# yweweler/single-speaker-tts

Hardware: AMD Instinct MI355X
Metric: mel-frames/sec (end-to-end text->waveform incl. 60-iter Griffin-Lim, 64-utt LJ-Speech-shaped batch per GPU) (higher is better)
Workload: dtype f32

## Files before the change

### include/sstts_hip.h

```cpp
#ifndef SSTTS_HIP_H
#define SSTTS_HIP_H

#include <stddef.h>
#include <stdint.h>

#ifdef __cplusplus
extern "C" {
#endif

typedef struct tts_handle_s* tts_handle_t;

enum tts_status {
    TTS_OK = 0,
    TTS_ERR_INVALID = -1,
    TTS_ERR_NOT_LOADED = -2,
    TTS_ERR_HIP = -3,
    TTS_ERR_DB_RANGE = -4,
    TTS_ERR_UNSUPPORTED = -5
};

typedef struct tts_config {
    int32_t struct_size;
    int32_t vocabulary_size;
    int32_t embedding_size;
    int32_t enc_prenet_units[2];
    int32_t enc_n_banks;
    int32_t enc_n_filters;
    int32_t enc_proj_filters[2];
    int32_t post_n_banks;
    int32_t post_n_filters;
    int32_t post_proj_filters[2];
    int32_t n_highway_layers;
    int32_t n_highway_units;
    int32_t n_gru_units;
    int32_t dec_prenet_units[2];
    int32_t n_attention_units;
    int32_t n_decoder_gru_units;
    int32_t n_decoder_gru_layers;
    int32_t n_mels;
    int32_t reduction;
    int32_t n_fft;
    int32_t force_cudnn;
    int32_t attention_mechanism;
    int32_t luong_local_window_d;
    int32_t luong_force_gaussian;
    int32_t luong_local_mode;
    int32_t apply_post_processing;
} tts_config_t;

enum tts_attention { TTS_ATTENTION_LUONG = 0, TTS_ATTENTION_LOCAL_LUONG = 1 };
enum tts_local_mode { TTS_LOCAL_MONOTONIC = 0, TTS_LOCAL_PREDICTIVE = 1 };

const char* tts_version(void);
int tts_default_config(tts_config_t* cfg);
int tts_create(const tts_config_t* cfg, int device_id, tts_handle_t* out);
int tts_destroy(tts_handle_t h);
const char* tts_last_error(tts_handle_t h);
int tts_set_stream(tts_handle_t h, void* hip_stream);
int tts_set_option(tts_handle_t h, const char* key, int value);
int tts_synchronize(tts_handle_t h);


int tts_manifest_size(tts_handle_t h);
int tts_manifest_entry(tts_handle_t h, int index, const char** name, int64_t shape[4], int* ndim);
int tts_set_weight(tts_handle_t h, const char* name, const float* host_data, const int64_t* shape, int ndim);
int tts_load_weights_blob(tts_handle_t h, const float* host_blob, size_t n_floats);
int tts_finalize_weights(tts_handle_t h);

int tts_malloc(void** dptr, size_t bytes);
int tts_free(void* dptr);
int tts_device_malloc(tts_handle_t h, void** dptr, size_t bytes);
int tts_device_free(tts_handle_t h, void* dptr);
int tts_memcpy_h2d(tts_handle_t h, void* dst, const void* src, size_t bytes);
int tts_memcpy_d2h(tts_handle_t h, void* dst, const void* src, size_t bytes);
int tts_memset(tts_handle_t h, void* dst, int value, size_t bytes);

int tts_encoder_forward(tts_handle_t h, const int32_t* ids, int B, int Ts, float* memory);
int tts_decoder_forward(tts_handle_t h, const float* memory, int B, int Ts, int n_steps,
                        float* mel, float* alignments);
int tts_postnet_forward(tts_handle_t h, const float* mel, int B, int T, float* linear);

int tts_evaluate(tts_handle_t h, const int32_t* ids, int B, int Ts, int n_steps,
                 const float* mel_target, const float* linear_target, float* losses,
                 double* l1_sums, float* mel, float* alignments, float* linear);

int tts_decoder_forward_teacher(tts_handle_t h, const float* memory, int B, int Ts, int n_steps,
                                const float* mel_target, float* mel, float* alignments);
int tts_teacher_forced(tts_handle_t h, const int32_t* ids, int B, int Ts, int n_steps,
                       const float* mel_target, const float* linear_target, float* losses,
                       double* l1_sums, float* mel, float* alignments, float* linear);
int tts_teacher_kernel_choice(tts_handle_t h, int B, int T_sent);

int tts_denorm_power(tts_handle_t h, const float* linear, int B, int T, int F,
                     float ref_db, float max_db, float power, float* mag);

int tts_griffin_lim(tts_handle_t h, const float* mag, const float* init_phase, uint64_t seed,
                    int B, int T, int n_iter, int win_length, int hop_length, int n_fft,
                    float* wav, float* mse);
int tts_griffin_lim_ragged(tts_handle_t h, const float* mag, const float* init_phase, uint64_t seed, int B, int T_max,
                           const int32_t* n_frames, int n_iter, int win_length, int hop_length, int n_fft,
                           float* wav, float* mse);
int tts_peak_normalize(tts_handle_t h, float* wav, int B, int n);

int tts_stft(tts_handle_t h, const float* wav, int B, int n, int n_fft, int win_length,
             int hop_length, float* out);
int tts_stft_magnitude(tts_handle_t h, const float* wav, int B, int n, int n_fft, int win_length,
                       int hop_length, float power, float* lin);
int tts_mel_spectrogram(tts_handle_t h, const float* lin, int B, int n_frames, int n_fft,
                        int sampling_rate, int n_mels, float fmin, float fmax, float* mel);
int tts_db_convert(tts_handle_t h, const float* in, size_t n, int mode, float ref_db, float max_db,
                   float* out);

int tts_trim_bounds(tts_handle_t h, const float* wav, const int64_t* offsets, int B, int frame_length, int hop_length,
                    float top_db, int64_t* bounds);

typedef struct tts_feature_params {
    int32_t struct_size;
    int32_t n_fft;
    int32_t win_length;
    int32_t hop_length;
    int32_t sampling_rate;
    int32_t n_mels;
    float fmin, fmax;
    float mel_ref_db, mel_max_db;
    float linear_ref_db, linear_max_db;
    int32_t normalize;
    int32_t reduction;
    int32_t trim;
    float trim_top_db;
    int32_t trim_frame_length;
    int32_t trim_hop_length;
} tts_feature_params_t;
int tts_default_feature_params(tts_feature_params_t* p);
int tts_plan_features(tts_handle_t h, const float* wav, const int64_t* offsets, int B, const tts_feature_params_t* p,
                      int64_t* plan);
int tts_extract_features(tts_handle_t h, const float* wav, const int64_t* offsets, int B, const tts_feature_params_t* p,
                         const int64_t* plan, float* mel_out, float* lin_out);

typedef struct tts_synth_params {
    int32_t n_steps;
    float ref_db, max_db;
    float power;
    int32_t n_iter;
    int32_t win_length, hop_length;
    uint64_t seed;
    int32_t peak_normalize;
    int32_t host_outputs;
} tts_synth_params_t;
#define TTS_HOST_LINEAR 1
#define TTS_HOST_ALIGNMENTS 2
int tts_synthesize(tts_handle_t h, const int32_t* ids, int B, int Ts, const tts_synth_params_t* p,
                   const float* init_phase , float* wav, float* mel,
                   float* alignments, float* linear);

int tts_synthesize_host(tts_handle_t h, const int32_t* ids_host, int B, int Ts, const tts_synth_params_t* p,
                        int* ticket);
int tts_wait_host(tts_handle_t h, int ticket, const float** wav_host, size_t* n_floats);
int tts_wait_host_outputs(tts_handle_t h, int ticket, const float** linear_host, size_t* n_linear, const float** align_host,
                          size_t* n_align);

int tts_profile_reset(tts_handle_t h);
int tts_decoder_kernel_choice(tts_handle_t h, int B, int T_sent, int pipelined);
int tts_debug_workspace(tts_handle_t h, const char* name, void** dptr, size_t* bytes);
int tts_debug_gl_plan(int T, int B, int win_length, int hop_length, int n_workers, int* items, int max_items, int* ring_frames);
int tts_debug_gl_plan_ragged(const int32_t* n_frames, int B, int win_length, int hop_length, int n_workers,
                             int* items, int max_items, int* ring_frames);
int tts_debug_gemm(tts_handle_t h, const float* A, const float* Wt, float* C, int M, int N, int Cin, int ktaps, int T,
                   int pool);
int tts_debug_hold(tts_handle_t h, int n_wgs, int lds_kb, double ms);
int tts_profile_get(tts_handle_t h, const char* stage, float* ms_total, int64_t* launches);
int tts_device_info(tts_handle_t h, char uuid_hex[33], int* n_compute_units);

#ifdef __cplusplus
}
#endif
#endif
```

### single-speaker-tts_amd/_hip.py

```python
import ctypes
import os
from ctypes import (POINTER, byref, c_char_p, c_float, c_int, c_int32, c_int64, c_size_t, c_uint64,
                    c_void_p)

import numpy as np

_HERE = os.path.dirname(os.path.abspath(__file__))
LIB_PATH = os.environ.get('SSTTS_HIP_LIB') or os.path.join(_HERE, 'libsstts_hip.so')

TTS_OK = 0
TTS_ERR_INVALID = -1
TTS_ERR_NOT_LOADED = -2
TTS_ERR_HIP = -3
TTS_ERR_DB_RANGE = -4
TTS_ERR_UNSUPPORTED = -5


class TtsError(RuntimeError):
    def __init__(self, code, msg):
        super().__init__('sstts_hip error {}: {}'.format(code, msg))
        self.code = code


class TtsConfig(ctypes.Structure):
    _fields_ = [
        ('struct_size', c_int32),
        ('vocabulary_size', c_int32), ('embedding_size', c_int32), ('enc_prenet_units', c_int32 * 2),
        ('enc_n_banks', c_int32), ('enc_n_filters', c_int32), ('enc_proj_filters', c_int32 * 2),
        ('post_n_banks', c_int32), ('post_n_filters', c_int32), ('post_proj_filters', c_int32 * 2),
        ('n_highway_layers', c_int32), ('n_highway_units', c_int32), ('n_gru_units', c_int32),
        ('dec_prenet_units', c_int32 * 2), ('n_attention_units', c_int32),
        ('n_decoder_gru_units', c_int32), ('n_decoder_gru_layers', c_int32), ('n_mels', c_int32),
        ('reduction', c_int32), ('n_fft', c_int32), ('force_cudnn', c_int32),
        ('attention_mechanism', c_int32), ('luong_local_window_d', c_int32), ('luong_force_gaussian', c_int32),
        ('luong_local_mode', c_int32), ('apply_post_processing', c_int32),
    ]


class TtsSynthParams(ctypes.Structure):
    _fields_ = [
        ('n_steps', c_int32), ('ref_db', c_float), ('max_db', c_float), ('power', c_float),
        ('n_iter', c_int32), ('win_length', c_int32), ('hop_length', c_int32), ('seed', c_uint64),
        ('peak_normalize', c_int32), ('host_outputs', c_int32),
    ]


class TtsFeatureParams(ctypes.Structure):
    _fields_ = [
        ('struct_size', c_int32), ('n_fft', c_int32), ('win_length', c_int32), ('hop_length', c_int32),
        ('sampling_rate', c_int32), ('n_mels', c_int32), ('fmin', c_float), ('fmax', c_float),
        ('mel_ref_db', c_float), ('mel_max_db', c_float), ('linear_ref_db', c_float), ('linear_max_db', c_float),
        ('normalize', c_int32), ('reduction', c_int32), ('trim', c_int32), ('trim_top_db', c_float),
        ('trim_frame_length', c_int32), ('trim_hop_length', c_int32),
    ]


_PROTOTYPES = {
    'tts_version': (c_char_p, []),
    'tts_default_config': (c_int, [POINTER(TtsConfig)]),
    'tts_create': (c_int, [POINTER(TtsConfig), c_int, POINTER(c_void_p)]),
    'tts_destroy': (c_int, [c_void_p]),
    'tts_last_error': (c_char_p, [c_void_p]),
    'tts_set_stream': (c_int, [c_void_p, c_void_p]),
    'tts_set_option': (c_int, [c_void_p, c_char_p, c_int]),
    'tts_synchronize': (c_int, [c_void_p]),
    'tts_manifest_size': (c_int, [c_void_p]),
    'tts_manifest_entry': (c_int, [c_void_p, c_int, POINTER(c_char_p), POINTER(c_int64), POINTER(c_int)]),
    'tts_set_weight': (c_int, [c_void_p, c_char_p, c_void_p, POINTER(c_int64), c_int]),
    'tts_load_weights_blob': (c_int, [c_void_p, c_void_p, c_size_t]),
    'tts_finalize_weights': (c_int, [c_void_p]),
    'tts_malloc': (c_int, [POINTER(c_void_p), c_size_t]),
    'tts_free': (c_int, [c_void_p]),
    'tts_device_malloc': (c_int, [c_void_p, POINTER(c_void_p), c_size_t]),
    'tts_device_free': (c_int, [c_void_p, c_void_p]),
    'tts_memcpy_h2d': (c_int, [c_void_p, c_void_p, c_void_p, c_size_t]),
    'tts_memcpy_d2h': (c_int, [c_void_p, c_void_p, c_void_p, c_size_t]),
    'tts_memset': (c_int, [c_void_p, c_void_p, c_int, c_size_t]),
    'tts_encoder_forward': (c_int, [c_void_p, c_void_p, c_int, c_int, c_void_p]),
    'tts_decoder_forward': (c_int, [c_void_p, c_void_p, c_int, c_int, c_int, c_void_p, c_void_p]),
    'tts_postnet_forward': (c_int, [c_void_p, c_void_p, c_int, c_int, c_void_p]),
    'tts_evaluate': (c_int, [c_void_p, c_void_p, c_int, c_int, c_int, c_void_p, c_void_p, c_void_p, c_void_p, c_void_p,
                             c_void_p, c_void_p]),
    'tts_decoder_forward_teacher': (c_int, [c_void_p, c_void_p, c_int, c_int, c_int, c_void_p, c_void_p, c_void_p]),
    'tts_teacher_forced': (c_int, [c_void_p, c_void_p, c_int, c_int, c_int, c_void_p, c_void_p, c_void_p, c_void_p,
                                   c_void_p, c_void_p, c_void_p]),
    'tts_teacher_kernel_choice': (c_int, [c_void_p, c_int, c_int]),
    'tts_denorm_power': (c_int, [c_void_p, c_void_p, c_int, c_int, c_int, c_float, c_float, c_float, c_void_p]),
    'tts_griffin_lim': (c_int, [c_void_p, c_void_p, c_void_p, c_uint64, c_int, c_int, c_int, c_int, c_int,
                                c_int, c_void_p, c_void_p]),
    'tts_griffin_lim_ragged': (c_int, [c_void_p, c_void_p, c_void_p, c_uint64, c_int, c_int, POINTER(c_int32), c_int, c_int,
                                       c_int, c_int, c_void_p, c_void_p]),
    'tts_peak_normalize': (c_int, [c_void_p, c_void_p, c_int, c_int]),
    'tts_stft': (c_int, [c_void_p, c_void_p, c_int, c_int, c_int, c_int, c_int, c_void_p]),
    'tts_db_convert': (c_int, [c_void_p, c_void_p, c_size_t, c_int, c_float, c_float, c_void_p]),
    'tts_stft_magnitude': (c_int, [c_void_p, c_void_p, c_int, c_int, c_int, c_int, c_int, c_float, c_void_p]),
    'tts_mel_spectrogram': (c_int, [c_void_p, c_void_p, c_int, c_int, c_int, c_int, c_int, c_float, c_float,
                                    c_void_p]),
    'tts_trim_bounds': (c_int, [c_void_p, c_void_p, c_void_p, c_int, c_int, c_int, c_float, c_void_p]),
    'tts_default_feature_params': (c_int, [POINTER(TtsFeatureParams)]),
    'tts_plan_features': (c_int, [c_void_p, c_void_p, c_void_p, c_int, POINTER(TtsFeatureParams), c_void_p]),
    'tts_extract_features': (c_int, [c_void_p, c_void_p, c_void_p, c_int, POINTER(TtsFeatureParams), c_void_p, c_void_p,
                                     c_void_p]),
    'tts_synthesize': (c_int, [c_void_p, c_void_p, c_int, c_int, POINTER(TtsSynthParams), c_void_p, c_void_p,
                               c_void_p, c_void_p, c_void_p]),
    'tts_synthesize_host': (c_int, [c_void_p, c_void_p, c_int, c_int, POINTER(TtsSynthParams), POINTER(c_int)]),
    'tts_wait_host': (c_int, [c_void_p, c_int, POINTER(c_void_p), POINTER(c_size_t)]),
    'tts_wait_host_outputs': (c_int, [c_void_p, c_int, POINTER(c_void_p), POINTER(c_size_t), POINTER(c_void_p), POINTER(c_size_t)]),
    'tts_profile_reset': (c_int, [c_void_p]),
    'tts_profile_get': (c_int, [c_void_p, c_char_p, POINTER(c_float), POINTER(c_int64)]),
    'tts_decoder_kernel_choice': (c_int, [c_void_p, c_int, c_int, c_int]),
    'tts_debug_workspace': (c_int, [c_void_p, c_char_p, POINTER(c_void_p), POINTER(c_size_t)]),
    'tts_debug_hold': (c_int, [c_void_p, c_int, c_int, ctypes.c_double]),
    'tts_debug_gemm': (c_int, [c_void_p, c_void_p, c_void_p, c_void_p, c_int, c_int, c_int, c_int, c_int, c_int]),
    'tts_debug_gl_plan': (c_int, [c_int, c_int, c_int, c_int, c_int, POINTER(c_int), c_int, POINTER(c_int)]),
    'tts_debug_gl_plan_ragged': (c_int, [POINTER(c_int32), c_int, c_int, c_int, c_int, POINTER(c_int), c_int, POINTER(c_int)]),
    'tts_device_info': (c_int, [c_void_p, c_char_p, POINTER(c_int)]),
}

_lib = None


def exported_symbols():
    return sorted(_PROTOTYPES)


def load_library(path=None):
    global _lib
    if _lib is not None and path is None:
        return _lib
    path = path or LIB_PATH
    if not os.path.exists(path):
        raise OSError('{} not found: build it with `python single-speaker-tts_amd/build.py` '
                      '(there is no CPU fallback)'.format(path))
    lib = ctypes.CDLL(path)
    for name, (res, args) in _PROTOTYPES.items():
        fn = getattr(lib, name)
        fn.restype = res
        fn.argtypes = args
    _lib = lib
    return lib


class DeviceArray(object):

    def __init__(self, engine, shape, dtype=np.float32):
        self.engine = engine
        self.shape = tuple(int(s) for s in shape)
        self.dtype = np.dtype(dtype)
        self.nbytes = int(np.prod(self.shape, dtype=np.int64)) * self.dtype.itemsize
        p = c_void_p()
        rc = engine.lib.tts_device_malloc(engine.handle, byref(p), self.nbytes)
        if rc != TTS_OK:
            raise TtsError(rc, 'tts_device_malloc({}) failed'.format(self.nbytes))
        self.ptr = p.value

    def data_ptr(self):
        return self.ptr

    def copy_from(self, host):
        host = np.ascontiguousarray(host, dtype=self.dtype)
        assert host.nbytes == self.nbytes, (host.shape, self.shape)
        self.engine._check(self.engine.lib.tts_memcpy_h2d(self.engine.handle, self.ptr, host.ctypes.data,
                                                          self.nbytes))
        return self

    def to_host(self):
        out = np.empty(self.shape, dtype=self.dtype)
        self.engine._check(self.engine.lib.tts_memcpy_d2h(self.engine.handle, out.ctypes.data, self.ptr,
                                                          self.nbytes))
        return out

    def free(self):
        if self.ptr:
            if getattr(self.engine, 'handle', None):
                self.engine.lib.tts_device_free(self.engine.handle, self.ptr)
            else:
                self.engine.lib.tts_free(self.ptr)
            self.ptr = None

    def __del__(self):
        try:
            self.free()
        except Exception:
            pass


def _is_device(x):
    return hasattr(x, 'data_ptr') and not isinstance(x, np.ndarray)


def ragged_frame_counts(n_frames, B, T_max, hop_length, n_fft):
    nf = np.ascontiguousarray(np.asarray(n_frames).reshape(-1), dtype=np.int32)
    if nf.shape[0] != B:
        raise ValueError('n_frames: {} lengths for a batch of {}'.format(nf.shape[0], B))
    for b, n in enumerate(nf.tolist()):
        if not 1 <= n <= T_max:
            raise ValueError('n_frames[{}] = {} is not in 1 .. T_max = {}'.format(b, n, T_max))
        if hop_length * (n - 1) <= n_fft // 2:
            raise ValueError('n_frames[{}] = {}: the signal is shorter than n_fft / 2 (reflect padding undefined)'.format(b, n))
    return nf


def momentum_thousandths(momentum):
    m = float(momentum)
    if not 0.0 <= m < 1.0:
        raise ValueError('momentum must be in [0, 1), got {!r}'.format(momentum))
    return min(999, int(round(m * 1000.0)))


class _MomentumScope(object):

    def __init__(self, engine, momentum):
        self.engine = engine
        self.value = None if momentum is None else momentum_thousandths(momentum)

    def __enter__(self):
        self.saved = self.engine._gl_momentum
        if self.value is not None and self.value != self.saved:
            self.engine.set_option('gl_momentum', self.value)

    def __exit__(self, *exc):
        if self.engine._gl_momentum != self.saved:
            self.engine.set_option('gl_momentum', self.saved)
        return False


class Engine(object):

    def __init__(self, hparams=None, device_id=0, stream=None):
        self.lib = load_library()
        cfg = TtsConfig()
        self.lib.tts_default_config(byref(cfg))
        if hparams is not None:
            enc, dec, post = hparams.encoder, hparams.decoder, hparams.post
            cfg.vocabulary_size = hparams.vocabulary_size
            cfg.embedding_size = enc.embedding_size
            cfg.enc_prenet_units[0], cfg.enc_prenet_units[1] = [l[0] for l in enc.pre_net_layers]
            cfg.enc_n_banks, cfg.enc_n_filters = enc.n_banks, enc.n_filters
            cfg.enc_proj_filters[0], cfg.enc_proj_filters[1] = [p[0] for p in enc.projections]
            cfg.post_n_banks, cfg.post_n_filters = post.n_banks, post.n_filters
            cfg.post_proj_filters[0], cfg.post_proj_filters[1] = [p[0] for p in post.projections]
            cfg.n_highway_layers, cfg.n_highway_units = enc.n_highway_layers, enc.n_highway_units
            cfg.n_gru_units = enc.n_gru_units
            cfg.dec_prenet_units[0], cfg.dec_prenet_units[1] = [l[0] for l in dec.pre_net_layers]
            cfg.n_attention_units = dec.n_attention_units
            cfg.n_decoder_gru_units = dec.n_decoder_gru_units
            cfg.n_decoder_gru_layers = dec.n_gru_layers
            cfg.n_mels, cfg.reduction, cfg.n_fft = hparams.n_mels, hparams.reduction, hparams.n_fft
            cfg.force_cudnn = 1 if hparams.force_cudnn else 0
            att = hparams.attention
            if att.mechanism not in ('LuongAttention', 'LocalLuongAttention'):
                raise NotImplementedError('attention mechanism {!r}'.format(att.mechanism))
            if att.mechanism == 'LocalLuongAttention' and (att.luong_local_mode not in ('monotonic', 'predictive') or
                                                           att.luong_local_score != 'dot'):
                raise NotImplementedError('LocalLuongAttention: the general / concat scores raise '
                                          'NotImplementedError in the reference too')
            cfg.luong_local_mode = 1 if att.luong_local_mode == 'predictive' else 0
            cfg.attention_mechanism = 1 if att.mechanism == 'LocalLuongAttention' else 0
            cfg.luong_local_window_d = att.luong_local_window_D
            cfg.luong_force_gaussian = 1 if att.luong_force_gaussian else 0
            cfg.apply_post_processing = 1 if hparams.apply_post_processing else 0
        self.cfg = cfg
        h = c_void_p()
        rc = self.lib.tts_create(byref(cfg), device_id, byref(h))
        if rc != TTS_OK:
            raise TtsError(rc, (self.lib.tts_last_error(None) or b'').decode())
        self.handle = h
# ... 412 lines not shown
```

### single-speaker-tts_amd/csrc/api_handle.hip

```cpp
#include "api_internal.h"

namespace tts_api {
thread_local std::string g_create_error;
const char* const kStageNames[ST_COUNT] = {"encoder", "decoder", "postnet", "denorm", "gl_iter", "gl_final", "debug_gemm", "eval_loss", "features"};
}

namespace tts_api {


int fail(tts_handle_t h, int code, const std::string& msg) {
    if (h) h->err = msg;
    else g_create_error = msg;
    return code;
}


const char* kAtt = "decoder2/decoder/output_projection_wrapper/multi_rnn_cell/cell_0/attention_wrapper";

const char* kMrc = "decoder2/decoder/output_projection_wrapper/multi_rnn_cell";


std::string bn_name(int i) {
    return i == 0 ? std::string("batch_normalization") : "batch_normalization_" + std::to_string(i);
}
// ... 179 lines not shown
        const auto& bh = W(h, hs + "/H/bias");
        const auto& bt = W(h, hs + "/T/bias");
        const size_t ow = p.alloc((size_t)2 * U * U);
        const size_t ob = p.alloc((size_t)2 * U);
        for (int u = 0; u < U; ++u) {
            const int s = u / 32, w = u % 32;
            const int rh = 64 * s + w, rt = 64 * s + 32 + w;
            for (int k = 0; k < U; ++k) {
                p.host[ow + (size_t)rh * U + k] = kh[(size_t)k * U + u];
                p.host[ow + (size_t)rt * U + k] = kt[(size_t)k * U + u];
            }
            p.host[ob + rh] = bh[u];
            p.host[ob + rt] = bt[u];
        }
        o.hw_wt.push_back(ow);
        o.hw_b.push_back(ob);
    }
    const int H = c.n_gru_units;
    o.gru_in_wt = p.alloc((size_t)6 * H * U);
    o.gru_in_b = p.alloc((size_t)6 * H);
    o.gru_rec = p.alloc(bigru_wrec_floats(H, cudnn));
    const size_t rec_stride = bigru_wrec_floats(H, cudnn) / 2;
    const char* dirs[2] = {"fw", "bw"};
    for (int d = 0; d < 2; ++d) {
        const std::string gs = scope + "/gru/" + dirs[d] + "/gru_cell_" + dirs[d];
        const auto& gk = W(h, gs + "/gates/kernel");
        const auto& gb = W(h, gs + "/gates/bias");
        const float* ck_in;
        int ck_in_ld;
        const float* ck_h;
        const float* cb;
        if (cudnn) {
            ck_in = W(h, gs + "/candidate/input_projection/kernel").data();
            ck_h = W(h, gs + "/candidate/hidden_projection/kernel").data();
            cb = W(h, gs + "/candidate/input_projection/bias").data();
        } else {
            ck_in = W(h, gs + "/candidate/kernel").data();
            ck_h = ck_in + (size_t)U * H;
            cb = W(h, gs + "/candidate/bias").data();
        }
        ck_in_ld = H;
        float* wt = p.host.data() + o.gru_in_wt + (size_t)d * 3 * H * U;
        float* bb = p.host.data() + o.gru_in_b + (size_t)d * 3 * H;
        for (int n = 0; n < 2 * H; ++n) {
            for (int k = 0; k < U; ++k) wt[(size_t)n * U + k] = gk[(size_t)k * 2 * H + n];
            bb[n] = gb[n];
        }
        for (int n = 0; n < H; ++n) {
            for (int k = 0; k < U; ++k) wt[(size_t)(2 * H + n) * U + k] = ck_in[(size_t)k * ck_in_ld + n];
            bb[2 * H + n] = cb[n];
        }
        float* rec = p.host.data() + o.gru_rec + (size_t)d * rec_stride;
        for (int k = 0; k < H; ++k)
            for (int n = 0; n < 2 * H; ++n) rec[(size_t)k * 2 * H + n] = gk[(size_t)(U + k) * 2 * H + n];
        float* rc = rec + (size_t)H * 2 * H;
        for (int k = 0; k < H; ++k)
            for (int n = 0; n < H; ++n) rc[(size_t)k * H + n] = ck_h[(size_t)k * H + n];
        if (cudnn) {
            const auto& hb = W(h, gs + "/candidate/hidden_projection/bias");
            for (int n = 0; n < H; ++n) rc[(size_t)H * H + n] = hb[n];
        }
    }
    return o;
}


void bind_cbhg(CbhgWeights& w, const CbhgOffsets& o, const float* base, int n_in, int n_banks, int n_filters,
               const int proj[2]) {
    w.n_banks = n_banks;
    w.n_filters = n_filters;
    w.c_in = n_in;
    w.proj_filters[0] = proj[0];
    w.proj_filters[1] = proj[1];
    for (int k = 0; k < n_banks; ++k) {
        w.bank_wt.push_back(base + o.bank_wt[k]);
        w.bank_b.push_back(base + o.bank_b[k]);
        w.bank_scale.push_back(base + o.bank_scale[k]);
        w.bank_shift.push_back(base + o.bank_shift[k]);
    }
    for (int i = 0; i < 2; ++i) {
        w.proj_wt[i] = base + o.proj_wt[i];
        w.proj_b[i] = base + o.proj_b[i];
        w.proj_scale[i] = base + o.proj_scale[i];
        w.proj_shift[i] = base + o.proj_shift[i];
    }
    w.lifter_wt = base + o.lifter_wt;
    w.lifter_b = base + o.lifter_b;
    for (size_t l = 0; l < o.hw_wt.size(); ++l) {
        w.hw_wt.push_back(base + o.hw_wt[l]);
        w.hw_b.push_back(base + o.hw_b[l]);
    }
    w.gru_in_wt = base + o.gru_in_wt;
    w.gru_in_b = base + o.gru_in_b;
    w.gru_rec = base + o.gru_rec;
}


struct GruOffsets {
    size_t gates_wt, gates_b, cand_wt, cand_b;
};


GruOffsets pack_dec_gru(tts_handle_t h, Packer& p, const std::string& scope, int n_in, int U, bool cudnn) {
    GruOffsets o{};
    const auto& gk = W(h, scope + "/gates/kernel");
    const auto& gb = W(h, scope + "/gates/bias");
    const int K = n_in + U;
    if (!cudnn) {
        o.gates_wt = pack_transposed(p, gk.data(), K, 2 * U);
        o.gates_b = pack_copy(p, gb.data(), 2 * U);
        o.cand_wt = pack_transposed(p, W(h, scope + "/candidate/kernel").data(), K, U);
        o.cand_b = pack_copy(p, W(h, scope + "/candidate/bias").data(), U);
        return o;
    }
    const auto& ik = W(h, scope + "/candidate/input_projection/kernel");
    const auto& ib = W(h, scope + "/candidate/input_projection/bias");
    const auto& hk = W(h, scope + "/candidate/hidden_projection/kernel");
    const auto& hb = W(h, scope + "/candidate/hidden_projection/bias");
    o.gates_wt = p.alloc((size_t)4 * U * K);
    o.gates_b = p.alloc((size_t)4 * U);
    float* wt = p.host.data() + o.gates_wt;
    float* bb = p.host.data() + o.gates_b;
    for (int n = 0; n < 2 * U; ++n) {
        for (int k = 0; k < K; ++k) wt[(size_t)n * K + k] = gk[(size_t)k * 2 * U + n];
        bb[n] = gb[n];
    }
    for (int n = 0; n < U; ++n) {
        for (int k = 0; k < U; ++k) wt[(size_t)(2 * U + n) * K + n_in + k] = hk[(size_t)k * U + n];
        bb[2 * U + n] = hb[n];
        for (int k = 0; k < n_in; ++k) wt[(size_t)(3 * U + n) * K + k] = ik[(size_t)k * U + n];
        bb[3 * U + n] = ib[n];
    }
    o.cand_wt = o.gates_wt;
    o.cand_b = o.gates_b;
    return o;
}


int pd_timed_out(tts_handle_t h) {
    return fail(h, TTS_ERR_HIP,
                "persistent decoder: a workgroup waited for its cluster longer than the bound (not all "
                "workgroups were co-resident); the outputs of that call are invalid -- the handle has "
                "switched to the launch-per-layer path (tts_set_option(h, \"persistent_decoder\", 1) switches back)");
}

int check_status(tts_handle_t h) {
    if (h->pd_used) {
        h->pd_used = false;
        int status = 0;
        HIPCHK(h, hipMemcpy(&status, h->pd_sync + 64 * h->pd_clusters + 1, sizeof(int), hipMemcpyDeviceToHost));
        if (status) HIPCHK(h, hipMemset(h->pd_sync + 64 * h->pd_clusters + 1, 0, sizeof(int)));
        if (status) h->persistent_decoder = 0;
        if (status) return pd_timed_out(h);
    }
    return TTS_OK;
}


int sync_all(tts_handle_t h) {
    HIPCHK(h, hipStreamSynchronize(h->stream));
    if (h->pl.front && h->pl.front != h->stream) HIPCHK(h, hipStreamSynchronize(h->pl.front));
    if (h->pl.aux) HIPCHK(h, hipStreamSynchronize(h->pl.aux));
    if (h->pl.encs) HIPCHK(h, hipStreamSynchronize(h->pl.encs));
    if (h->hio.out) HIPCHK(h, hipStreamSynchronize(h->hio.out));
    return check_status(h);
}


int graph_quiesce(tts_handle_t h) {
    HIPCHK(h, h->graph_done.sync());
    h->graph_done.disarm();
    return TTS_OK;
}

int graph_drop(tts_handle_t h) {
    if (h->dec_graph) {
        int rc = graph_quiesce(h);
        if (rc) return rc;
        hipGraphExecDestroy(h->dec_graph);
        h->dec_graph = nullptr;
    }
    if (h->dec_graph_src) {
        hipGraphDestroy(h->dec_graph_src);
        h->dec_graph_src = nullptr;
    }
    return TTS_OK;
}


int ws_get(tts_handle_t h, const char* name, size_t bytes, void** out) {
    DevBuf& b = h->ws[name];
    if (b.bytes < bytes) {
        if (b.p) {
            {
                int rc = sync_all(h);
                if (rc) return rc;
            }
            HIPCHK(h, hipFree(b.p));
            b.p = nullptr;
            b.bytes = 0;
            {
                int rc = graph_drop(h);
                if (rc) return rc;
            }
        }
        HIPCHK(h, hipMalloc(&b.p, bytes));
        b.bytes = bytes;
    }
    *out = b.p;
    return TTS_OK;
}


void prof_collect(tts_handle_t h) {
    sync_all(h);
    if (!h->spans.empty() && h->debug_hooks && h->timeline) {
        for (auto& s : h->spans) {
            float t0 = 0.f, t1 = 0.f;
            if (hipEventElapsedTime(&t0, h->spans[0].a, s.a) == hipSuccess &&
                hipEventElapsedTime(&t1, h->spans[0].a, s.b) == hipSuccess)
                fprintf(stderr, "timeline %-8s %9.3f -> %9.3f ms (%.3f)\n", kStageNames[s.stage], t0, t1, t1 - t0);
        }
    }
    for (auto& s : h->spans) {
        float ms = 0.f;
        if (hipEventElapsedTime(&ms, s.a, s.b) == hipSuccess) {
            h->prof_ms[s.stage] += ms;
            h->prof_launches[s.stage] += s.launches;
        }
        hipEventDestroy(s.a);
        hipEventDestroy(s.b);
    }
    h->spans.clear();
}


GemmGroup dense_group(const float* A, int lda, const float* Wt, const float* bias, float* C, int ldc, int M, int N,
                      int K, int act) {
    GemmGroup g;
    std::memset(&g, 0, sizeof(g));
    g.A = A; g.Wt = Wt; g.bias = bias; g.C = C;
    g.M = M; g.N = N; g.K = K;
    g.lda = lda; g.T = M; g.Cin = K; g.padl = 0; g.pool = 0;
    g.ldc = ldc; g.coff = 0; g.act = act; g.epi = EPI_STD;
    return g;
}


GemmGroup conv_group(const float* A, int Cin, int ktaps, int T, const float* Wt, const float* bias,
                     const float* scale, const float* shift, float* C, int ldc, int coff, int M, int N, int act,
                     int pool) {
    GemmGroup g;
    std::memset(&g, 0, sizeof(g));
    g.A = A; g.Wt = Wt; g.bias = bias; g.scale = scale; g.shift = shift; g.C = C;
    g.M = M; g.N = N; g.K = ktaps * Cin;
    g.lda = Cin; g.T = T; g.Cin = Cin; g.padl = (ktaps - 1) / 2; g.pool = pool;
    g.ldc = ldc; g.coff = coff; g.act = act; g.epi = EPI_STD;
    return g;
}


int run_single(tts_handle_t h, const GemmGroup& g) {
    GemmBatch b;
    std::memset(&b, 0, sizeof(b));
    b.g[0] = g;
    HIPCHK(h, launch_gemm(h->stream, b, 1));
    return TTS_OK;
}


bool graph_runtime_ok(int* have) {
    int v = 0;
    if (hipRuntimeGetVersion(&v) != hipSuccess) v = 0;
    if (have) *have = v;
    return v / 100000 >= HIP_VERSION / 100000;
}

}

extern "C" {


const char* tts_version(void) { return "sstts_hip 0.1.0 (gfx950)"; }


int tts_default_config(tts_config_t* c) {
    if (!c) return TTS_ERR_INVALID;
    std::memset(c, 0, sizeof(*c));
    c->struct_size = (int32_t)sizeof(tts_config_t);
    c->vocabulary_size = 39;
    c->embedding_size = 256;
    c->enc_prenet_units[0] = 256; c->enc_prenet_units[1] = 128;
    c->enc_n_banks = 16; c->enc_n_filters = 128;
    c->enc_proj_filters[0] = 128; c->enc_proj_filters[1] = 128;
    c->post_n_banks = 8; c->post_n_filters = 128;
    c->post_proj_filters[0] = 256; c->post_proj_filters[1] = 80;
    c->n_highway_layers = 4; c->n_highway_units = 128; c->n_gru_units = 128;
    c->dec_prenet_units[0] = 256; c->dec_prenet_units[1] = 128;
    c->n_attention_units = 256; c->n_decoder_gru_units = 256; c->n_decoder_gru_layers = 2;
    c->n_mels = 80; c->reduction = 5; c->n_fft = 2048; c->force_cudnn = 0;
    c->attention_mechanism = TTS_ATTENTION_LUONG;
    c->luong_local_window_d = 10;
    c->luong_force_gaussian = 1;
    c->luong_local_mode = TTS_LOCAL_MONOTONIC;
    c->apply_post_processing = 1;
    return TTS_OK;
// ... 20 lines not shown
        !mult(c.enc_n_filters, 32) || !mult(c.post_n_filters, 32) || !mult(c.enc_proj_filters[0], 4) ||
        !mult(c.post_proj_filters[0], 4))
        return fail(nullptr, TTS_ERR_UNSUPPORTED, "layer widths must be multiples of 16 (filters: 32)");
    if (c.enc_proj_filters[1] != c.enc_prenet_units[1] || c.post_proj_filters[1] != c.n_mels)
        return fail(nullptr, TTS_ERR_INVALID, "last projection must match the CBHG input width (residual)");
    if (c.attention_mechanism != TTS_ATTENTION_LUONG && c.attention_mechanism != TTS_ATTENTION_LOCAL_LUONG)
        return fail(nullptr, TTS_ERR_UNSUPPORTED, "attention_mechanism must be TTS_ATTENTION_LUONG or TTS_ATTENTION_LOCAL_LUONG");
    if (c.attention_mechanism == TTS_ATTENTION_LOCAL_LUONG && c.luong_local_window_d < 1)
        return fail(nullptr, TTS_ERR_INVALID, "luong_local_window_d must be >= 1");
    if (c.luong_local_mode != TTS_LOCAL_MONOTONIC && c.luong_local_mode != TTS_LOCAL_PREDICTIVE)
        return fail(nullptr, TTS_ERR_INVALID, "luong_local_mode must be TTS_LOCAL_MONOTONIC or TTS_LOCAL_PREDICTIVE");
    if (c.enc_n_banks < 1 || c.post_n_banks < 1 || c.reduction < 1 || c.vocabulary_size < 1 || c.n_highway_layers < 0)
        return fail(nullptr, TTS_ERR_INVALID, "bad counts");
    if (c.n_mels > TTS_MAX_N_MELS)
        return fail(nullptr, TTS_ERR_UNSUPPORTED,
                    "n_mels is " + std::to_string(c.n_mels) + ", at most " + std::to_string(TTS_MAX_N_MELS) +
                    " supported (the decoder's GO frame is read from a block of that many zeros)");
    {
        const int fields[] = {c.vocabulary_size, c.embedding_size, c.enc_prenet_units[0], c.enc_prenet_units[1], c.enc_n_banks,
                              c.enc_n_filters, c.enc_proj_filters[0], c.enc_proj_filters[1], c.post_n_banks, c.post_n_filters,
                              c.post_proj_filters[0], c.post_proj_filters[1], c.dec_prenet_units[0], c.dec_prenet_units[1],
                              c.reduction, c.n_highway_layers};
        for (int v : fields)
            if (v > TTS_MAX_FIELD)
                return fail(nullptr, TTS_ERR_UNSUPPORTED, "a count or layer width of " + std::to_string(v) + ": at most " +
                                                              std::to_string(TTS_MAX_FIELD) + " (2^20) supported");
        struct { const char* what; long long n; } mats[] = {
            {"the embedding table (vocabulary_size x embedding_size)", (long long)c.vocabulary_size * c.embedding_size},
            {"encoder pre-net layer 1", (long long)c.embedding_size * c.enc_prenet_units[0]},
            {"encoder pre-net layer 2", (long long)c.enc_prenet_units[0] * c.enc_prenet_units[1]},
            {"the widest encoder bank convolution (enc_n_banks x enc_prenet_units[1] x enc_n_filters)",
             (long long)c.enc_n_banks * c.enc_prenet_units[1] * c.enc_n_filters},
            {"encoder projection 1 (3 x enc_n_banks x enc_n_filters x enc_proj_filters[0])",
             3ll * c.enc_n_banks * c.enc_n_filters * c.enc_proj_filters[0]},
            {"encoder projection 2", 3ll * c.enc_proj_filters[0] * c.enc_proj_filters[1]},
            {"the widest post-net bank convolution (post_n_banks x n_mels x post_n_filters)",
             c.apply_post_processing ? (long long)c.post_n_banks * c.n_mels * c.post_n_filters : 0},
            {"post-net projection 1 (3 x post_n_banks x post_n_filters x post_proj_filters[0])",
             c.apply_post_processing ? 3ll * c.post_n_banks * c.post_n_filters * c.post_proj_filters[0] : 0},
            {"post-net projection 2", c.apply_post_processing ? 3ll * c.post_proj_filters[0] * c.post_proj_filters[1] : 0},
            {"the output projection (n_decoder_gru_units x n_mels x reduction)",
             (long long)c.n_decoder_gru_units * c.n_mels * c.reduction}};
        for (const auto& m : mats)
            if (m.n > TTS_MAX_WEIGHT_FLOATS)
                return fail(nullptr, TTS_ERR_UNSUPPORTED,
                            std::string(m.what) + " has " + std::to_string(m.n) + " weights, at most " +
                            std::to_string(TTS_MAX_WEIGHT_FLOATS) + " (2^30 - 5) supported: the GEMM loaders address an operand "
                            "with 32-bit byte offsets");
    }
    if (hipSetDevice(device_id) != hipSuccess) return fail(nullptr, TTS_ERR_HIP, "hipSetDevice failed");
    auto h = new tts_handle_s();
    h->cfg = c;
    h->device = device_id;
    if (hipStreamCreate(&h->stream) != hipSuccess) {
        delete h;
        return fail(nullptr, TTS_ERR_HIP, "hipStreamCreate failed");
    }
    h->own_stream = true;
    {
        int cus = 0;
        if (hipDeviceGetAttribute(&cus, hipDeviceAttributeMultiprocessorCount, device_id) != hipSuccess || cus < 1) cus = 256;
        h->n_cus_dev = cus;
    }
    build_manifest(h);
    *out = h;
    return TTS_OK;
}


int tts_destroy(tts_handle_t h) {
    DeviceScope dev_scope(h);
    if (!h) return TTS_OK;
    hipSetDevice(h->device);
    hipStreamSynchronize(h->stream);
    for (auto& s : h->spans) {
        hipEventDestroy(s.a);
        hipEventDestroy(s.b);
    }
    graph_drop(h);
    for (auto& kv : h->ws)
        if (kv.second.p) hipFree(kv.second.p);
    if (h->arena) hipFree(h->arena);
    if (h->gl.window) hipFree(h->gl.window);
    if (h->gl.wss) hipFree(h->gl.wss);
    if (h->gl.wlane) hipFree(h->gl.wlane);
    if (h->gl.tw1024) hipFree(h->gl.tw1024);
    if (h->gl.tw2048) hipFree(h->gl.tw2048);
    if (h->gl.tables) hipFree(h->gl.tables);
    if (h->an.window) hipFree(h->an.window);
    if (h->an.mel_wt) hipFree(h->an.mel_wt);
    feat_release(h);
    if (h->an.flag) hipFree(h->an.flag);
    for (auto& kv : h->glg.tw) hipFree(kv.second);
    if (h->glg.window) hipFree(h->glg.window);
    if (h->glg.rwss) hipFree(h->glg.rwss);
    h->pl.teardown();
    h->hio.teardown();
    if (h->own_stream) hipStreamDestroy(h->stream);
    delete h;
    return TTS_OK;
}


const char* tts_last_error(tts_handle_t h) { return h ? h->err.c_str() : g_create_error.c_str(); }


int tts_set_stream(tts_handle_t h, void* s) {
    DeviceScope dev_scope(h);
    if (!h) return TTS_ERR_INVALID;
    {
        int rc = sync_all(h);
        if (rc) return rc;
    }
    h->pl.reset();
    {
        int rc = graph_drop(h);
        if (rc) return rc;
    }
    if (h->own_stream) hipStreamDestroy(h->stream);
    if (s) {
        h->stream = reinterpret_cast<hipStream_t>(s);
        h->own_stream = false;
    } else {
        HIPCHK(h, hipStreamCreate(&h->stream));
        h->own_stream = true;
    }
    return TTS_OK;
}


int tts_set_option(tts_handle_t h, const char* key, int value) {
    DeviceScope dev_scope(h);
    if (!h || !key) return TTS_ERR_INVALID;
    if (!std::strcmp(key, "use_graph")) {
        int have = 0;
        if (value && !(value == 2 && h->debug_hooks) && !graph_runtime_ok(&have))
            return fail(h, TTS_ERR_UNSUPPORTED,
                        "use_graph: this process runs the library on HIP runtime " + std::to_string(have) + ", older than the " +
                        std::to_string(HIP_VERSION) + " it was built with (a libamdhip64 loaded before the library, e.g. the one "
                        "PyTorch bundles); hipGraph replays of the decoder are wrong there (csrc/api_internal.h, `use_graph`) -- the "
                        "launches are enqueued directly instead");
        h->use_graph = value;
    }
    else if (!std::strcmp(key, "profile")) h->profile = value;
    else if (!std::strcmp(key, "fused_tail")) h->fused_tail = value;
    else if (!std::strcmp(key, "persistent_decoder")) {
        if (value != h->persistent_decoder) {
            int rc = sync_all(h);
            if (rc) return rc;
        }
        h->persistent_decoder = value;
    }
    else if (!std::strcmp(key, "gl_pair")) h->gl_pair = value;
    else if (!std::strcmp(key, "gl_momentum")) {
        if (value < 0 || value > 999) return fail(h, TTS_ERR_INVALID, "gl_momentum: thousandths of the momentum, 0 .. 999");
        h->gl_momentum = value;
    }
    else if (!std::strcmp(key, "gl_wide_from")) h->gl_wide = value < -2 ? -2 : value;
    else if (!std::strcmp(key, "pd_ws")) {
        if (value != h->pd_ws) {
            int rc = sync_all(h);
            if (rc) return rc;
        }
        h->pd_ws = value;
    }
    else if (!std::strcmp(key, "enc_stream")) {
        int rc = sync_all(h);
        if (rc) return rc;
        h->enc_stream = value;
    }
    else if (!std::strcmp(key, "debug_hooks")) h->debug_hooks = value;
    else if (!std::strcmp(key, "pd_debug_delay") || !std::strcmp(key, "gl_runs") || !std::strcmp(key, "gl_run_len") ||
             !std::strcmp(key, "timeline") || !std::strcmp(key, "gl_workers") || !std::strcmp(key, "pd_rows")) {
        if (!h->debug_hooks && value != 0)
            return fail(h, TTS_ERR_INVALID, std::string(key) + ": a test hook; set the option \"debug_hooks\" to 1 on this handle first");
        if (!std::strcmp(key, "pd_debug_delay")) h->pd_debug_delay = value;
        else if (!std::strcmp(key, "gl_runs")) h->gl_runs = value;
        else if (!std::strcmp(key, "gl_run_len")) h->gl_run_len = value;
        else if (!std::strcmp(key, "gl_workers")) h->gl_workers = value;
        else if (!std::strcmp(key, "pd_rows")) h->pd_rows = value;
        else h->timeline = value;
    }
    else if (!std::strcmp(key, "reserve_cus")) {
        if (value != h->reserve_cus) {
            int rc = sync_all(h);
            if (rc) return rc;
        }
        h->reserve_cus = value;
    } else if (!std::strcmp(key, "hold_lds_kb")) {
        if (value < 1 || value > 160) return fail(h, TTS_ERR_INVALID, "hold_lds_kb must be 1..160");
        h->hold_lds_kb = value;
    } else if (!std::strcmp(key, "pipeline")) {
        int rc = sync_all(h);
        if (rc) return rc;
        h->pl.reset();
        h->pipeline = value;
    }
    else return fail(h, TTS_ERR_INVALID, std::string("unknown option ") + key);
    return TTS_OK;
}


int tts_synchronize(tts_handle_t h) {
    DeviceScope dev_scope(h);
    if (!h) return TTS_ERR_INVALID;
    return sync_all(h);
}


int tts_manifest_size(tts_handle_t h) { return h ? (int)h->manifest.size() : TTS_ERR_INVALID; }


int tts_manifest_entry(tts_handle_t h, int i, const char** name, int64_t shape[4], int* ndim) {
    if (!h || i < 0 || i >= (int)h->manifest.size()) return TTS_ERR_INVALID;
    const auto& e = h->manifest[i];
    if (name) *name = e.name.c_str();
    if (ndim) *ndim = (int)e.shape.size();
    if (shape)
        for (size_t d = 0; d < 4; ++d) shape[d] = d < e.shape.size() ? e.shape[d] : 1;
    return TTS_OK;
}


int tts_set_weight(tts_handle_t h, const char* name, const float* data, const int64_t* shape, int ndim) {
    if (!h || !name || !data || !shape) return TTS_ERR_INVALID;
    for (const auto& e : h->manifest) {
        if (e.name != name) continue;
        if ((int)e.shape.size() != ndim) return fail(h, TTS_ERR_INVALID, std::string("rank mismatch for ") + name);
        for (int d = 0; d < ndim; ++d)
            if (e.shape[d] != shape[d]) return fail(h, TTS_ERR_INVALID, std::string("shape mismatch for ") + name);
        h->host_w[e.name].assign(data, data + e.numel());
        h->finalized = false;
        return TTS_OK;
    }
    return fail(h, TTS_ERR_INVALID, std::string("unknown weight ") + name);
}


int tts_load_weights_blob(tts_handle_t h, const float* blob, size_t n) {
    if (!h || !blob) return TTS_ERR_INVALID;
    size_t total = 0;
    for (const auto& e : h->manifest) total += e.numel();
    if (total != n)
        return fail(h, TTS_ERR_INVALID,
                    "blob has " + std::to_string(n) + " floats, manifest needs " + std::to_string(total));
    size_t off = 0;
    for (const auto& e : h->manifest) {
        h->host_w[e.name].assign(blob + off, blob + off + e.numel());
        off += e.numel();
    }
    h->finalized = false;
    return TTS_OK;
}


int tts_finalize_weights(tts_handle_t h) {
    DeviceScope dev_scope(h);
    if (!h) return TTS_ERR_INVALID;
    for (const auto& e : h->manifest)
        if (!h->host_w.count(e.name)) return fail(h, TTS_ERR_NOT_LOADED, "missing weight " + e.name);
    HIPCHK(h, hipSetDevice(h->device));
    const tts_config_t& c = h->cfg;
    const bool cudnn = c.force_cudnn != 0;
    Packer p;
    const size_t o_emb = pack_copy(p, W(h, "encoder/embedding").data(), (size_t)c.vocabulary_size * c.embedding_size);
    size_t o_epw[2], o_epb[2];
    int n_in = c.embedding_size;
    for (int i = 0; i < 2; ++i) {
        const std::string s = "encoder/pre_net/" + std::to_string(i + 1) + "-FC-" + std::to_string(c.enc_prenet_units[i]);
        o_epw[i] = pack_transposed(p, W(h, s + "/kernel").data(), n_in, c.enc_prenet_units[i]);
        o_epb[i] = pack_copy(p, W(h, s + "/bias").data(), c.enc_prenet_units[i]);
        n_in = c.enc_prenet_units[i];
    }
    const CbhgOffsets o_enc =
        pack_cbhg(h, p, "encoder", n_in, c.enc_n_banks, c.enc_n_filters, c.enc_proj_filters, cudnn);
    const int mem = 2 * c.n_gru_units, att = c.n_attention_units, U = c.n_decoder_gru_units;
    const size_t o_mem = pack_transposed(p, W(h, "decoder2/memory_layer/kernel").data(), mem, att);
    size_t o_dpw[2], o_dpb[2];
    n_in = c.n_mels + att;
    for (int i = 0; i < 2; ++i) {
        const std::string s = std::string(kAtt) + "/pre_net/" + std::to_string(i + 1) + "-FC-" +
                              std::to_string(c.dec_prenet_units[i]);
        o_dpw[i] = pack_transposed(p, W(h, s + "/kernel").data(), n_in, c.dec_prenet_units[i]);
        o_dpb[i] = pack_copy(p, W(h, s + "/bias").data(), c.dec_prenet_units[i]);
        n_in = c.dec_prenet_units[i];
    }
    size_t o_dpfw, o_dpfb;
    {
        const int NM = c.n_mels, OUTW = c.n_mels * c.reduction, P1 = c.dec_prenet_units[0];
        const std::string s1 = std::string(kAtt) + "/pre_net/1-FC-" + std::to_string(P1);
        const auto& w1 = W(h, s1 + "/kernel");
        const auto& b1 = W(h, s1 + "/bias");
        const auto& wo = W(h, "decoder2/decoder/output_projection_wrapper/kernel");
        const auto& bo = W(h, "decoder2/decoder/output_projection_wrapper/bias");
        const int K = U + att;
        o_dpfw = p.alloc((size_t)P1 * K);
        o_dpfb = p.alloc((size_t)P1);
        for (int n = 0; n < P1; ++n) {
            for (int k = 0; k < U; ++k) {
                double acc = 0.0;
                for (int j = 0; j < NM; ++j)
                    acc += (double)wo[(size_t)k * OUTW + (OUTW - NM) + j] * (double)w1[(size_t)j * P1 + n];
                p.host[o_dpfw + (size_t)n * K + k] = (float)acc;
            }
            for (int k = 0; k < att; ++k) p.host[o_dpfw + (size_t)n * K + U + k] = w1[(size_t)(NM + k) * P1 + n];
            double bacc = (double)b1[n];
            for (int j = 0; j < NM; ++j) bacc += (double)bo[(OUTW - NM) + j] * (double)w1[(size_t)j * P1 + n];
            p.host[o_dpfb + n] = (float)bacc;
        }
    }
    const GruOffsets o_ag = pack_dec_gru(h, p, std::string(kAtt) + "/gru_cell", n_in, att, cudnn);
    const size_t o_al = pack_transposed(p, W(h, std::string(kAtt) + "/attention_layer/kernel").data(), att + mem, att);
    const bool predictive = c.attention_mechanism == TTS_ATTENTION_LOCAL_LUONG && c.luong_local_mode == TTS_LOCAL_PREDICTIVE;
    size_t o_wp = 0, o_vp = 0;
    if (predictive) {
        o_wp = pack_copy(p, W(h, std::string(kAtt) + "/local_luong_attention/local_w_p").data(), (size_t)att * att);
        o_vp = pack_copy(p, W(h, std::string(kAtt) + "/local_luong_attention/local_v_p").data(), (size_t)att);
    }
    GruOffsets o_dg[4];
    for (int i = 0; i < c.n_decoder_gru_layers; ++i)
        o_dg[i] = pack_dec_gru(h, p, std::string(kMrc) + "/cell_" + std::to_string(i + 1) + "/gru_cell",
                               i == 0 ? att : U, U, cudnn);
    const int OUT = c.n_mels * c.reduction;
    const size_t o_ow = pack_transposed(p, W(h, "decoder2/decoder/output_projection_wrapper/kernel").data(), U, OUT);
    const size_t o_ob = pack_copy(p, W(h, "decoder2/decoder/output_projection_wrapper/bias").data(), OUT);
    CbhgOffsets o_post{};
    if (c.apply_post_processing)
        o_post = pack_cbhg(h, p, "post_process", c.n_mels, c.post_n_banks, c.post_n_filters, c.post_proj_filters, cudnn);
    const int F = 1 + c.n_fft / 2;
    const size_t o_dw = pack_transposed(p, W(h, "dense/kernel").data(), c.apply_post_processing ? mem : c.n_mels, F);
    const size_t o_db = pack_copy(p, W(h, "dense/bias").data(), F);
    const size_t o_zero = p.alloc(TTS_MAX_N_MELS);
    size_t o_wsw = 0, o_wsb = 0;
// ... 177 lines not shown
```

### single-speaker-tts_amd/csrc/api_internal.h

```cpp
#pragma once
#include <cmath>
#include <cstdio>
#include <cstring>
#include <memory>
#include <mutex>
#include <optional>
#include <string>
#include <utility>
#include <vector>
#include "decoder.h"
#include "griffin_lim.h"
#include "tts_common.h"
#include <algorithm>
#include <map>

namespace tts_api {
using namespace tts;


constexpr int TTS_MAX_N_MELS = 1024;
constexpr int TTS_MAX_FIELD = 1 << 20;
constexpr long long TTS_MAX_WEIGHT_FLOATS = (1ll << 30) - 5;

extern thread_local std::string g_create_error;
// ... 30 lines not shown
    hipEvent_t a, b;
    int stage;
    int64_t launches;
};

struct Signal {
    hipEvent_t ev = nullptr;
    bool armed = false;
    Signal() = default;
    Signal(const Signal&) = delete;
    Signal& operator=(const Signal&) = delete;
    ~Signal() {
        if (ev) hipEventDestroy(ev);
    }
    hipError_t record(hipStream_t s) {
        hipError_t e = ev ? hipSuccess : hipEventCreateWithFlags(&ev, hipEventDisableTiming);
        if (e == hipSuccess) e = hipEventRecord(ev, s);
        if (e == hipSuccess) armed = true;
        return e;
    }
    hipError_t wait(hipStream_t s) const { return armed ? hipStreamWaitEvent(s, ev, 0) : hipSuccess; }
    hipError_t sync() const { return armed ? hipEventSynchronize(ev) : hipSuccess; }
    void disarm() { armed = false; }
};

template <class T>
struct StagedBuf {
    T* pinned = nullptr;
    T* dev = nullptr;
    size_t bytes = 0;
    StagedBuf() = default;
    StagedBuf(const StagedBuf&) = delete;
    StagedBuf& operator=(const StagedBuf&) = delete;
    ~StagedBuf() { release(); }
    hipError_t release() {
        const hipError_t e1 = pinned ? hipHostFree(pinned) : hipSuccess;
        const hipError_t e2 = dev ? hipFree(dev) : hipSuccess;
        pinned = dev = nullptr;
        bytes = 0;
        return e1 != hipSuccess ? e1 : e2;
    }
    hipError_t grow(size_t need) {
        if (need <= bytes) return hipSuccess;
        hipError_t e = release();
        if (e == hipSuccess) e = hipHostMalloc(reinterpret_cast<void**>(&pinned), need, hipHostMallocDefault);
        if (e == hipSuccess) e = hipMalloc(reinterpret_cast<void**>(&dev), need);
        if (e == hipSuccess) bytes = need;
        return e;
    }
};

struct StageArgs {
    int* hold_flag = nullptr;
    int cu_budget = 0;
    bool chip_idle = false;
    bool project_later = false;
    int parity = 0;
    float* keys = nullptr;
    struct {
        int32_t* dst = nullptr;
        const int32_t* src = nullptr;
        size_t bytes = 0;
        Signal* done = nullptr;
    } upload;
    Signal* enc_done = nullptr;
};

struct CallPipeline {
    hipStream_t aux = nullptr;
    int* hold_flags = nullptr;
    Signal aux_mark;
    unsigned call_count = 0;
    hipStream_t front = nullptr;
    hipStream_t encs = nullptr;
    Signal enc_ready[2];
    Signal dec_done[2];
    Signal gap[2];
    Signal front_done;
    Signal post_done[2];
    bool gl_wide_used[2] = {false, false};
    Signal gl_done[2];
    Signal serial_done;
    unsigned syn_calls = 0;
    int syn_shape[3] = {0, 0, 0};
    int last_enc_ahead = -1;

    void reset() {
        for (Signal* s : {&aux_mark, &front_done, &serial_done}) s->disarm();
        for (int i = 0; i < 2; ++i) {
            for (Signal* s : {&enc_ready[i], &dec_done[i], &gap[i], &post_done[i], &gl_done[i]}) s->disarm();
            gl_wide_used[i] = false;
        }
    }
    void teardown() {
        for (hipStream_t s : {front, aux})
            if (s) {
                hipStreamSynchronize(s);
                hipStreamDestroy(s);
            }
        if (hold_flags) hipFree(hold_flags);
        if (encs) hipStreamDestroy(encs);
    }
};

struct HostIo {
    hipStream_t out = nullptr;
    StagedBuf<int32_t> ids[3];
    StagedBuf<float> wav[3];
    Signal h2d[3];
    Signal enc[3];
    Signal ready[3];
    Signal d2h[3];
    size_t n_floats[3] = {0, 0, 0};
    StagedBuf<float> lin[3], ali[3];
    size_t n_lin[3] = {0, 0, 0}, n_ali[3] = {0, 0, 0};
    bool failed[3] = {false, false, false};
    int* status_pinned = nullptr;
    int tickets = 0;

    void reset() {
        for (int i = 0; i < 3; ++i)
            for (Signal* s : {&h2d[i], &enc[i], &ready[i], &d2h[i]}) s->disarm();
    }
    void teardown() {
        if (status_pinned) hipHostFree(status_pinned);
        if (out) hipStreamDestroy(out);
    }
};

}
using namespace tts_api;

struct tts_handle_s {
    tts_config_t cfg;
    int device = 0;
    hipStream_t stream = nullptr;
    bool own_stream = false;
    std::string err;
    int use_graph = 0;
    int fused_tail = 1;
    bool tail_configured = false;
    int profile = 0;
    int pipeline = 1;
    int reserve_cus = 32;
    int hold_lds_kb = 64;
    int enc_stream = 1;
    CallPipeline pl;
    int persistent_decoder = 1;
    int pd_ws = 1;
    bool ws_configured = false;
    int gl_pair = 3;
    int gl_momentum = 0;
    int gl_wide = -1;
    int n_cus_dev = 0;
    bool pd_configured = false;
    int debug_hooks = 0;
    int pd_debug_delay = 0;
    int gl_runs = 0;
    int gl_run_len = 0;
    int timeline = 0;
    int gl_workers = 0;
    unsigned* gl_ring = nullptr;
    unsigned gl_ring_seq = 0;
    unsigned* gl_ring_last = nullptr;
    hipStream_t gl_ring_stream = nullptr;
    bool pd_used = false;
    unsigned* pd_sync = nullptr;
    int pd_clusters = 0;
    int pd_rows = 0;
    int pd_rows_used = 0;

    HostIo hio;

    std::vector<ManifestEntry> manifest;
    std::map<std::string, std::vector<float>> host_w;
    bool finalized = false;

    float* arena = nullptr;
    size_t arena_floats = 0;

    const float* embedding = nullptr;
    const float* enc_pre_wt[2];
    const float* enc_pre_b[2];
    CbhgWeights enc, post;
    const float* mem_wt = nullptr;
    DecoderWeights dec;
    const float* dense_wt = nullptr;
    const float* dense_b = nullptr;
    const float* zeros = nullptr;

    std::map<std::string, DevBuf> ws;

    hipGraphExec_t dec_graph = nullptr;
    Signal graph_done;
    hipGraph_t dec_graph_src = nullptr;
    struct {
        const void* memory = nullptr;
        const void* keys = nullptr;
        void* align = nullptr;
        int B = 0, Ts = 0, n_steps = 0;
        DecoderScratch sc;
        DecoderWeights w;
    } dec_key;

    struct {
        int win = 0, hop = 0, T = 0;
        float* window = nullptr;
        float* wss = nullptr;
        float* wlane = nullptr;
        float2* tw1024 = nullptr;
        float2* tw2048 = nullptr;
        float2* tables = nullptr;
        bool configured = false;
        int n_cus = 0;
    } gl;

    struct {
        std::map<int, float2*> tw;
        int n_fft = 0, win = 0, hop = 0, T = 0;
        float* window = nullptr;
        float* rwss = nullptr;
        bool configured = false;
    } glg;

    struct {
        std::vector<int> tab_key, plan_key;
        int* lens = nullptr;
        float* rw = nullptr;
        int4* items = nullptr;
        int n_items = 0, slots = 1, workers = 1;
    } rag;

    struct {
        int win = 0;
        float* window = nullptr;
        int sr = 0, n_fft = 0, n_mels = 0;
        float fmin = 0, fmax = 0;
        float* mel_wt = nullptr;
        int* flag = nullptr;
    } an;

    struct {
        int n_fft = 0, win = 0;
        float* window = nullptr;
        int sr = 0, n_mels = 0;
        float fmin = 0, fmax = 0;
        float* mel_w = nullptr;
        int* mel_band = nullptr;
        void* staging = nullptr;
        size_t staging_bytes = 0;
        Signal staged;
    } feat;

    std::vector<ProfSpan> spans;
    double prof_ms[ST_COUNT] = {0};
    int64_t prof_launches[ST_COUNT] = {0};
};


namespace tts_api {

#define HIPCHK(h, expr)                                                                         \
    do {                                                                                        \
        hipError_t _e = (expr);                                                                 \
        if (_e != hipSuccess) {                                                                 \
            (h)->err = std::string(#expr) + ": " + hipGetErrorString(_e);                       \
            return TTS_ERR_HIP;                                                                 \
        }                                                                                       \
    } while (0)

struct DeviceScope {
    int prev = -1;
    bool changed = false;
    explicit DeviceScope(tts_handle_t h) {
        if (!h) return;
        if (hipGetDevice(&prev) == hipSuccess && prev != h->device) changed = hipSetDevice(h->device) == hipSuccess;
    }
    ~DeviceScope() {
        if (changed) hipSetDevice(prev);
    }
    DeviceScope(const DeviceScope&) = delete;
    DeviceScope& operator=(const DeviceScope&) = delete;
};

#define WS(h, name, type, count, var)                                             \
    type* var = nullptr;                                                          \
    {                                                                             \
        void* _p = nullptr;                                                       \
        int _rc = ws_get(h, name, (size_t)(count) * sizeof(type), &_p);           \
        if (_rc != TTS_OK) return _rc;                                            \
        var = reinterpret_cast<type*>(_p);                                        \
    }

struct ProfScope {
    tts_handle_t h;
    int idx = -1;
    ProfScope(tts_handle_t h_, int stage, int64_t launches) : h(h_) {
        if (!h->profile) return;
        ProfSpan s{};
        if (hipEventCreate(&s.a) != hipSuccess || hipEventCreate(&s.b) != hipSuccess) return;
        s.stage = stage;
        s.launches = launches;
        hipEventRecord(s.a, h->stream);
        h->spans.push_back(s);
        idx = (int)h->spans.size() - 1;
    }
    ~ProfScope() {
        if (idx >= 0) hipEventRecord(h->spans[idx].b, h->stream);
    }
};

int fail(tts_handle_t h, int code, const std::string& msg);
void build_manifest(tts_handle_t h);
int pd_timed_out(tts_handle_t h);
// ... 41 lines not shown
```

### single-speaker-tts_amd/csrc/api_stages.hip

```cpp
#include "api_internal.h"

namespace tts_api {


int run_cbhg(tts_handle_t h, const CbhgWeights& w, const char* tag, const float* x, int B, int T, float* out,
             int64_t* launches) {
    const tts_config_t& c = h->cfg;
    const int M = B * T;
    const int NB = w.n_banks, NF = w.n_filters;
    const int U = c.n_highway_units, H = c.n_gru_units;
    const std::string t(tag);
    WS(h, (t + ".bank").c_str(), float, (size_t)M * NB * NF, bank);
    WS(h, (t + ".p1").c_str(), float, (size_t)M * w.proj_filters[0], p1);
    WS(h, (t + ".p2").c_str(), float, (size_t)M * w.proj_filters[1], p2);
    WS(h, (t + ".hw0").c_str(), float, (size_t)M * U, hw0);
    WS(h, (t + ".hw1").c_str(), float, (size_t)M * U, hw1);
    WS(h, (t + ".xproj").c_str(), float, (size_t)M * 6 * H, xproj);

    for (int k0 = 0; k0 < NB; k0 += TTS_GEMM_MAX_GROUPS) {
        GemmBatch b;
        std::memset(&b, 0, sizeof(b));
        const int ng = std::min(TTS_GEMM_MAX_GROUPS, NB - k0);
        for (int i = 0; i < ng; ++i) {
            const int k = k0 + ng - 1 - i;
// ... 335 lines not shown
        rwss = h->rag.rw;
    }
    const float2* tw = nullptr;
    if ((rc = glg_twiddles(h, n_fft, &tw))) return rc;
    const int F = 1 + n_fft / 2, Fp = gl_fp(n_fft), L = hop * (T - 1);
    WS(h, "glg.phase", float2, (size_t)B * T * Fp, ph);
    WS(h, "glg.frames", float, (size_t)B * T * win, frames);
    WS(h, "glg.mse_partial", float, (size_t)B * T, msep);
    const float alpha = (float)(h->gl_momentum / 1000.0);
    float2* mom_c = nullptr;
    if (h->gl_momentum > 0 && n_iter > 1) {
        WS(h, "glg.mom", float2, (size_t)B * T * Fp, mc);
        mom_c = mc;
    }
    float* sig = wav;
    HIPCHK(h, launch_glg_phase_init(h->stream, init_ft, seed, ph, B, F, T, Fp, d_lens));
    {
        ProfScope ps(h, ST_GL_ITER, 3 * (int64_t)n_iter);
        for (int it = 0; it < n_iter; ++it) {
            HIPCHK(h, launch_glg_istft(h->stream, mag_int, ph, h->glg.window, rwss, tw, frames, sig, B, T, Fp, n_fft, win, hop, d_lens));
            const bool want_mse = mse && it == n_iter - 1;
            HIPCHK(h, launch_glg_stft(h->stream, sig, L, h->glg.window, tw, ph, B, T, Fp, n_fft, win, hop, 0, mag_int,
                                      want_mse ? msep : nullptr, mom_c, alpha, it == 0, d_lens));
        }
    }
    if (mse) {
        if (n_iter > 0 && d_lens) HIPCHK(h, launch_gl_mse_reduce_ragged(h->stream, msep, B, T, F, d_lens, 1, mse));
        else if (n_iter > 0) HIPCHK(h, launch_gl_mse_reduce(h->stream, msep, B, T, (float)((double)F * T), mse));
        else HIPCHK(h, hipMemsetAsync(mse, 0, B * sizeof(float), h->stream));
    }
    {
        ProfScope ps(h, ST_GL_FINAL, 2);
        HIPCHK(h, launch_glg_istft(h->stream, mag_int, ph, h->glg.window, rwss, tw, frames, wav, B, T, Fp, n_fft, win, hop, d_lens));
    }
    if (peak_normalize) HIPCHK(h, launch_peak_normalize(h->stream, wav, B, L));
    return TTS_OK;
}


int gl_prepare(tts_handle_t h, int T, int win, int hop, int n_fft) {
    if (!gl_is_streaming(n_fft, win, hop)) return fail(h, TTS_ERR_UNSUPPORTED, "griffin_lim: the streaming kernel is instantiated for 1102 / 275 and 800 / 200 at n_fft 2048 only");
    if (win < 2 || win > n_fft || hop < 1 || T < 1)
        return fail(h, TTS_ERR_INVALID, "griffin_lim: need 2 <= win_length <= n_fft, hop_length >= 1, T >= 1");
    const int ncol = (win + hop - 1) / hop;
    if (ncol > 8) return fail(h, TTS_ERR_UNSUPPORTED, "griffin_lim: win_length / hop_length > 8 not supported");
    if ((long long)hop * (T - 1) <= n_fft / 2)
        return fail(h, TTS_ERR_INVALID, "griffin_lim: signal shorter than n_fft/2 (reflect padding undefined)");
    auto& g = h->gl;
    {
        int rc = gl_tables(h);
        if (rc) return rc;
    }
    if (g.win == win && g.hop == hop && g.T == T) return TTS_OK;
    HIPCHK(h, hipStreamSynchronize(h->stream));
    if (g.window) hipFree(g.window);
    if (g.wss) hipFree(g.wss);
    if (g.wlane) hipFree(g.wlane);
    g.window = g.wss = g.wlane = nullptr;
    std::vector<double> wd;
    std::vector<float> wf, wss;
    hann_window(win, wd, wf);
    recip_window_sumsquare(wd, n_fft, hop, T, wss);
    HIPCHK(h, hipMalloc(&g.window, win * sizeof(float)));
    HIPCHK(h, hipMalloc(&g.wss, wss.size() * sizeof(float)));
    HIPCHK(h, hipMemcpy(g.window, wf.data(), win * sizeof(float), hipMemcpyHostToDevice));
    HIPCHK(h, hipMemcpy(g.wss, wss.data(), wss.size() * sizeof(float), hipMemcpyHostToDevice));
    {
        std::vector<float> wl(2 * 16 * 2 * 64);
        gl_build_wlane(wf.data(), wss.data(), win, hop, T, wl.data());
        HIPCHK(h, hipMalloc(&g.wlane, wl.size() * sizeof(float)));
        HIPCHK(h, hipMemcpy(g.wlane, wl.data(), wl.size() * sizeof(float), hipMemcpyHostToDevice));
    }
    g.win = win;
    g.hop = hop;
    g.T = T;
    return TTS_OK;
}


int gl_run(tts_handle_t h, const float* mag_int, const float* init_ft, uint64_t seed, int B, int T, int n_iter,
           int win, int hop, int n_fft, float* wav, float* mse, bool peak_normalize,
           bool under_reservation, float2* const* phase_pair, bool phase_ready,
           int wide_from, const int32_t* n_frames) {
    int rc = gl_prepare(h, T, win, hop, n_fft);
    if (rc) return rc;
    if (n_frames) {
        if (peak_normalize || under_reservation || phase_pair)
            return fail(h, TTS_ERR_INVALID, "griffin_lim: a ragged batch is a stand-alone call without peak normalisation");
        if ((rc = gl_rag_tables(h, n_frames, B, T, win, hop, n_fft, true))) return rc;
    }
    const int F = 1 + n_fft / 2, FP = TTS_GL_FP;
    float2 *ph0, *ph1;
    if (phase_pair) {
        ph0 = phase_pair[0]; ph1 = phase_pair[1];
    } else {
        WS(h, "gl.phase0", unsigned, (size_t)B * T * FP * (gl_state_bytes() / sizeof(unsigned)), own0);
        WS(h, "gl.phase1", unsigned, (size_t)B * T * FP * (gl_state_bytes() / sizeof(unsigned)), own1);
        ph0 = reinterpret_cast<float2*>(own0); ph1 = reinterpret_cast<float2*>(own1);
    }
    GlParams p;
    std::memset(&p, 0, sizeof(p));
    p.mag = mag_int;
    p.window = h->gl.window;
    p.rwss = h->gl.wss;
    p.wlane = h->gl.wlane;
    p.tw1024 = h->gl.tw1024;
    p.tw2048 = h->gl.tw2048;
    p.tables = h->gl.tables;
    p.T = T; p.FP = FP; p.win = win; p.hop = hop;
    p.ncol = (win + hop - 1) / hop;
    p.B = B;
    if (n_frames) {
        p.n_frames = h->rag.lens;
        p.rw_edge = h->rag.rw;
        p.rw_E = gl_rw_edge_len(n_fft, win, hop);
    }
    if (gl_stream_ring_frames(win, hop) < 1)
        return fail(h, TTS_ERR_UNSUPPORTED, "griffin_lim: this window / hop pair does not fit the LDS ring (hop beyond the window's 128-sample slots, or too long)");
    const int n_cus = (h->debug_hooks && h->gl_workers >= 16 && h->gl_workers <= device_cus(h)) ? h->gl_workers : device_cus(h);
    const int held = (under_reservation && h->reserve_cus > 0) ? h->reserve_cus : 0;
    int per_launch = h->gl_pair;
    per_launch = per_launch < 1 ? 1 : (per_launch > 3 ? 3 : per_launch);
    while (per_launch > 1 && gl_stream_ring_frames(win, hop, per_launch) <= 0) --per_launch;
    if (h->gl_momentum > 0 && n_iter > 1) {
        WS(h, "gl.mom", float2, (size_t)B * T * FP, mc);
        p.mom_c = mc;
        p.mom_alpha = (float)(h->gl_momentum / 1000.0);
        per_launch = 1;
    }
    if (n_frames) {
        if ((rc = gl_rag_plan(h, p, n_frames, n_cus, per_launch, h->debug_hooks ? h->gl_runs : 0, h->debug_hooks ? h->gl_run_len : 0))) return rc;
    } else
    HIPCHK(h, gl_plan_stream(p, n_cus - held > 16 ? n_cus - held : n_cus, per_launch, h->debug_hooks ? h->gl_runs : 0,
                             h->debug_hooks ? h->gl_run_len : 0, h->stream));
    GlParams pw = p;
    const bool two_cuts = held > 0 && wide_from >= 0 && n_cus - held > 16 &&
                          !(h->debug_hooks && (h->gl_runs || h->gl_run_len));
    if (two_cuts) HIPCHK(h, gl_plan_stream(pw, n_cus, per_launch, 0, 0, h->stream));
    const int nchunks = std::max(p.slots_per_utt, pw.slots_per_utt);
    WS(h, "gl.mse_partial", float, (size_t)B * ((p.mom_c && mse) ? std::max(nchunks, T) : nchunks), msep);
    constexpr unsigned GL_RING = 256;
    WS(h, "gl.counter_ring", unsigned, GL_RING, ring);
    if (ring != h->gl_ring || h->gl_ring_stream != h->stream) {
        HIPCHK(h, hipMemsetAsync(ring, 0, GL_RING * sizeof(unsigned), h->stream));
        h->gl_ring = ring;
        h->gl_ring_stream = h->stream;
        h->gl_ring_last = nullptr;
    }
    auto next_counter = [&](GlParams& q) {
        q.clear_counter = h->gl_ring_last;
        q.work_counter = ring + (h->gl_ring_seq++ % GL_RING);
        h->gl_ring_last = q.work_counter;
    };
    const bool seed_in_kernel = !init_ft && n_iter >= 1;
    if (!phase_ready && !seed_in_kernel) HIPCHK(h, launch_phase_init(h->stream, init_ft, seed, ph0, B, F, T, FP, p.n_frames));
    p.F = pw.F = F;
    p.seed = pw.seed = seed;
    int launch_idx = 0, mse_chunks = p.slots_per_utt, peak_chunks = p.slots_per_utt;
    float2* cur = ph0;
    float2* nxt = ph1;
    const int free_cus = n_cus - held > 16 ? n_cus - held : n_cus;
    {
        ProfScope ps(h, ST_GL_ITER, n_iter);
        for (int it = 0; it < n_iter;) {
            const bool want_mse = mse && it == n_iter - 1;
            const int left = n_iter - (mse ? 1 : 0) - it;
            const int n_stage = left >= per_launch ? per_launch : (left >= 1 ? left : 1);
            const bool wide = two_cuts && launch_idx >= wide_from;
            GlParams& q = wide ? pw : p;
            q.phase_in = cur;
            q.phase_out = nxt;
            q.seeded = seed_in_kernel && it == 0;
            q.mom_first = it == 0;
            q.mse_partial = want_mse ? msep : nullptr;
            if (want_mse) mse_chunks = q.mom_c ? T : q.slots_per_utt;
            next_counter(q);
            HIPCHK(h, launch_gl_stream(h->stream, q, wide ? n_cus : free_cus, 0, n_stage));
            std::swap(cur, nxt);
            it += n_stage;
            ++launch_idx;
        }
    }
    if (mse) {
        if (n_iter > 0 && n_frames) {
            HIPCHK(h, launch_gl_mse_reduce_ragged(h->stream, msep, B, mse_chunks, F, p.n_frames, p.mom_c ? 1 : 0, mse));
        } else if (n_iter > 0) {
            HIPCHK(h, launch_gl_mse_reduce(h->stream, msep, B, mse_chunks, (float)((double)F * T), mse));
        } else {
            HIPCHK(h, hipMemsetAsync(mse, 0, B * sizeof(float), h->stream));
        }
    }
    {
        ProfScope ps(h, ST_GL_FINAL, 1);
        const bool wide = two_cuts && launch_idx >= wide_from;
        GlParams& q = wide ? pw : p;
        q.seeded = 0;
        q.phase_in = cur;
        q.phase_out = nullptr;
        q.mse_partial = nullptr;
        q.wav = wav;
        q.peak_partial = peak_normalize ? msep : nullptr;
        if (n_frames && !gl_rag_all_full(n_frames, B, T)) HIPCHK(h, hipMemsetAsync(wav, 0, (size_t)B * hop * (T - 1) * sizeof(float), h->stream));
        next_counter(q);
        HIPCHK(h, launch_gl_stream(h->stream, q, wide ? n_cus : free_cus, 1, 1));
        peak_chunks = q.slots_per_utt;
    }
    if (peak_normalize) HIPCHK(h, launch_peak_scale(h->stream, wav, B, hop * (T - 1), msep, peak_chunks));
    return TTS_OK;
}


int standalone_begin(tts_handle_t h) {
    if (!h->pl.encs) return TTS_OK;
    for (int i = 0; i < 2; ++i) {
        HIPCHK(h, h->pl.enc_ready[i].wait(h->stream));
        HIPCHK(h, h->pl.dec_done[i].wait(h->stream));
    }
    return TTS_OK;
}

int standalone_end(tts_handle_t h) {
    if (h->pl.front) HIPCHK(h, h->pl.serial_done.record(h->stream));
    return TTS_OK;
}

int encoder_impl(tts_handle_t h, const int32_t* ids, int B, int Ts, float* memory) {
    int rc = TTS_OK;
    const tts_config_t& c = h->cfg;
    const int M = B * Ts;
    WS(h, "enc.pre1", float, (size_t)M * c.enc_prenet_units[0], pre1);
    WS(h, "enc.pre2", float, (size_t)M * c.enc_prenet_units[1], pre2);
    int64_t launches = 0;
    ProfScope ps(h, ST_ENCODER, 0);
    {
        GemmGroup g = dense_group(h->embedding, c.embedding_size, h->enc_pre_wt[0], h->enc_pre_b[0], pre1,
                                  c.enc_prenet_units[0], M, c.enc_prenet_units[0], c.embedding_size, ACT_RELU);
        g.gather = ids;
        g.gather_rows = c.vocabulary_size;
        if ((rc = run_single(h, g))) return rc;
    }
    if ((rc = run_single(h, dense_group(pre1, c.enc_prenet_units[0], h->enc_pre_wt[1], h->enc_pre_b[1], pre2,
                                        c.enc_prenet_units[1], M, c.enc_prenet_units[1], c.enc_prenet_units[0],
                                        ACT_RELU))))
        return rc;
    launches += 2;
    if ((rc = run_cbhg(h, h->enc, "enc", pre2, B, Ts, memory, &launches))) return rc;
    if (ps.idx >= 0) h->spans[ps.idx].launches = launches;
    return TTS_OK;
}


int pd_kernel_for(tts_handle_t h, int B, int Ts, int budget) {
    const int cudnn = h->cfg.force_cudnn;
    if (h->pd_ws && decoder_ws_supports(h->dec, cudnn, B, Ts) && decoder_ws_workgroups(B) <= budget) return 2;
    if (decoder_persistent_supports(h->dec, cudnn, B, Ts) && decoder_persistent_workgroups(B) <= budget) return 1;
    return 0;
}


int pd_choice(tts_handle_t h, int B, int Ts, int budget, bool pipelined) {
    if (h->persistent_decoder <= 0) return 0;
    const int k = pd_kernel_for(h, B, Ts, budget);
    if (h->persistent_decoder >= 2) return k;
    if (k == 2) return 2;
    if (k == 1) return (pipelined && B > 48) ? 1 : 0;
    return 0;
}


int attention_keys(tts_handle_t h, const float* memory, int B, int Ts, float* keys) {
    const int A = h->cfg.n_attention_units, mem = 2 * h->cfg.n_gru_units;
    return run_single(h, dense_group(memory, mem, h->mem_wt, nullptr, keys, A, B * Ts, A, mem, ACT_NONE));
}

int teacher_choice(tts_handle_t h, int B, int Ts) {
    return pd_choice(h, B, Ts, h->n_cus_dev, false) == 2 && h->dec.ws_teacher ? 2 : 0;
}

int decoder_impl(tts_handle_t h, const float* memory, int B, int Ts, int n_steps, float* mel, float* alignments,
                 const float* target, const StageArgs& args, std::optional<GemmGroup>* deferred) {
    int rc = TTS_OK;
    const tts_config_t& c = h->cfg;
    if (h->dec.local_d > 0 && Ts < 2 * h->dec.local_d + 1)
        return fail(h, TTS_ERR_UNSUPPORTED,
                    "LocalLuongAttention: the memory must hold at least 2*D+1 positions (for shorter inputs the reference pads "
                    "the window's 2D+1 alignments to 4D+2-T_s entries, tacotron/attention.py:294-299,85-92: its attention state "
                    "changes shape and TensorFlow fails)");
    const int A = c.n_attention_units, U = c.n_decoder_gru_units, mem = 2 * c.n_gru_units;
    const int NL = c.n_decoder_gru_layers;
    WS(h, "dec.keys", float, (size_t)B * Ts * A, keys_ws);
    float* keys = args.keys ? args.keys : keys_ws;
    const bool have_keys = args.keys != nullptr;
    const size_t state_floats = (size_t)B * (A + 2 * ((size_t)A + (size_t)NL * U));
    WS(h, "dec.state", float, state_floats, state);
    WS(h, "dec.tmp", float, (size_t)B * (c.dec_prenet_units[0] + c.dec_prenet_units[1] + 6 * (size_t)U), tmp);
    WS(h, "dec.ctx_parts", float, (size_t)TTS_ATT_PARTS * B * mem, ctx_parts);
    WS(h, "dec.att_stats", float, (size_t)n_steps * B * TTS_ATT_PARTS * 2, att_stats);
    const int pd_budget = args.cu_budget > 0 ? args.cu_budget : h->n_cus_dev;
    const int pd_kernel = target ? teacher_choice(h, B, Ts) : pd_choice(h, B, Ts, pd_budget, args.cu_budget > 0);
    const bool use_pd = pd_kernel != 0;
    const bool defer_proj = args.project_later && deferred && use_pd && !target;
    WS(h, defer_proj ? (args.parity ? "dec.yhist.odd" : "dec.yhist.even") : "dec.yhist", float, (size_t)B * n_steps * U, yhist);
    WS(h, "dec.align_raw", float, (size_t)n_steps * B * Ts, align_raw);
    DecoderScratch sc;
    std::memset(&sc, 0, sizeof(sc));
    sc.state = state;
    sc.state_bytes = state_floats * sizeof(float);
    sc.att = state;
    sc.h_att = state + (size_t)B * A;
    for (int l = 0; l < NL; ++l) sc.h_dec[l] = state + (size_t)B * (2 * A + (size_t)l * U);
    {
        float* alt = state + (size_t)B * (2 * A + (size_t)NL * U);
        sc.h_att_alt = alt;
        for (int l = 0; l < NL; ++l) sc.h_dec_alt[l] = alt + (size_t)B * (A + (size_t)l * U);
    }
    float* t = tmp;
    sc.p1 = t; t += (size_t)B * c.dec_prenet_units[0];
    sc.p2 = t; t += (size_t)B * c.dec_prenet_units[1];
    sc.rh = t; t += (size_t)B * U;
    sc.u = t; t += (size_t)B * U;
    sc.hh = t; t += (size_t)B * U;
    sc.xi = t; t += (size_t)B * U;
    sc.y0 = t; t += (size_t)B * U;
    sc.y1 = t; t += (size_t)B * U;
    sc.ctx_parts = ctx_parts;
    sc.att_stats = att_stats;
    sc.yhist = yhist;
    sc.align_raw = align_raw;
// ... 344 lines not shown
        if (T < 1 || win_length < 2 || win_length > n_fft || hop_length < 1)
            return fail(h, TTS_ERR_INVALID, "griffin_lim: need 2 <= win_length <= n_fft, hop_length >= 1, T >= 1");
        const int Fg = 1 + n_fft / 2, Fp = gl_fp(n_fft);
        WS(h, "gl.mag", float, (size_t)B * T * Fp, magg);
        HIPCHK(h, launch_mag_ft_to_tf(h->stream, mag, magg, B, Fg, T, Fp));
        return gl_run_generic(h, magg, init_phase, seed, B, T, n_iter, win_length, hop_length, n_fft, wav, mse, false);
    }
    int rc = gl_prepare(h, T, win_length, hop_length, n_fft);
    if (rc) return rc;
    const int F = 1 + n_fft / 2, FP = TTS_GL_FP;
    WS(h, "gl.mag", float, (size_t)B * T * FP, magi);
    HIPCHK(h, launch_mag_ft_to_tf(h->stream, mag, magi, B, F, T, FP));
    return gl_run(h, magi, init_phase, seed, B, T, n_iter, win_length, hop_length, n_fft, wav, mse);
}


int tts_griffin_lim_ragged(tts_handle_t h, const float* mag, const float* init_phase, uint64_t seed, int B, int T_max,
                           const int32_t* n_frames, int n_iter, int win_length, int hop_length, int n_fft, float* wav, float* mse) {
    DeviceScope dev_scope(h);
    if (!h || !mag || !wav || !n_frames || B < 1 || n_iter < 0) return fail(h, TTS_ERR_INVALID, "griffin_lim_ragged: bad arguments");
    const bool streaming = gl_is_streaming(n_fft, win_length, hop_length);
    if (!streaming && !glg_supports(n_fft)) return fail(h, TTS_ERR_UNSUPPORTED, "griffin_lim: n_fft must be a power of two between 256 and 4096");
    if (T_max < 1 || win_length < 2 || win_length > n_fft || hop_length < 1)
        return fail(h, TTS_ERR_INVALID, "griffin_lim: need 2 <= win_length <= n_fft, hop_length >= 1, T >= 1");
    for (int b = 0; b < B; ++b) {
        if (n_frames[b] < 1 || n_frames[b] > T_max)
            return fail(h, TTS_ERR_INVALID, "griffin_lim_ragged: n_frames[" + std::to_string(b) + "] = " + std::to_string(n_frames[b]) +
                                                " is not in 1 .. T_max = " + std::to_string(T_max));
        if ((long long)hop_length * (n_frames[b] - 1) <= n_fft / 2)
            return fail(h, TTS_ERR_INVALID, "griffin_lim_ragged: utterance " + std::to_string(b) + " (" + std::to_string(n_frames[b]) +
                                                " frames): signal shorter than n_fft/2 (reflect padding undefined)");
    }
    const int F = 1 + n_fft / 2, Fp = streaming ? TTS_GL_FP : gl_fp(n_fft);
    int rc = streaming ? gl_prepare(h, T_max, win_length, hop_length, n_fft) : TTS_OK;
    if (rc) return rc;
    if ((rc = gl_rag_tables(h, n_frames, B, T_max, win_length, hop_length, n_fft, streaming))) return rc;
    WS(h, "gl.mag", float, (size_t)B * T_max * Fp, magi);
    HIPCHK(h, launch_mag_ft_to_tf(h->stream, mag, magi, B, F, T_max, Fp, h->rag.lens));
    if (!streaming) return gl_run_generic(h, magi, init_phase, seed, B, T_max, n_iter, win_length, hop_length, n_fft, wav, mse, false, n_frames);
    return gl_run(h, magi, init_phase, seed, B, T_max, n_iter, win_length, hop_length, n_fft, wav, mse, false, false, nullptr, false, -1, n_frames);
}


int tts_peak_normalize(tts_handle_t h, float* wav, int B, int n) {
    DeviceScope dev_scope(h);
    if (!h || !wav || B < 1 || n < 1) return fail(h, TTS_ERR_INVALID, "peak_normalize: bad arguments");
    HIPCHK(h, launch_peak_normalize(h->stream, wav, B, n));
    return TTS_OK;
}


int tts_stft(tts_handle_t h, const float* wav, int B, int n, int n_fft, int win_length, int hop_length, float* out) {
    DeviceScope dev_scope(h);
    if (!h || !wav || !out || B < 1) return fail(h, TTS_ERR_INVALID, "stft: bad arguments");
    float2* buf;
    int Tf;
    int rc = stft_run(h, wav, B, n, n_fft, win_length, hop_length, &buf, &Tf);
    if (rc) return rc;
    HIPCHK(h, launch_cplx_tf_to_ft(h->stream, buf, out, B, 1 + n_fft / 2, Tf, gl_fp(n_fft), 0, 1.0f));
    return TTS_OK;
}


int tts_stft_magnitude(tts_handle_t h, const float* wav, int B, int n, int n_fft, int win_length, int hop_length,
                       float power, float* lin) {
    DeviceScope dev_scope(h);
    if (!h || !wav || !lin || B < 1) return fail(h, TTS_ERR_INVALID, "stft_magnitude: bad arguments");
    float2* buf;
    int Tf;
    int rc = stft_run(h, wav, B, n, n_fft, win_length, hop_length, &buf, &Tf);
    if (rc) return rc;
    HIPCHK(h, launch_cplx_tf_to_ft(h->stream, buf, lin, B, 1 + n_fft / 2, Tf, gl_fp(n_fft), 1, power));
    return TTS_OK;
}


int tts_mel_spectrogram(tts_handle_t h, const float* lin, int B, int n_frames, int n_fft, int sr, int n_mels, float fmin,
                        float fmax, float* mel) {
    DeviceScope dev_scope(h);
    if (!h || !lin || !mel || B < 1 || n_frames < 1 || n_mels < 1 || sr < 1)
        return fail(h, TTS_ERR_INVALID, "mel_spectrogram: bad arguments");
    if (n_fft < 2 || (n_fft & 1)) return fail(h, TTS_ERR_INVALID, "mel_spectrogram: n_fft must be even");
    const int F = 1 + n_fft / 2, FP = gl_fp(n_fft);
    auto& a = h->an;
    if (!a.mel_wt || a.sr != sr || a.n_fft != n_fft || a.n_mels != n_mels || a.fmin != fmin || a.fmax != fmax) {
        auto hz2mel = [](double f) { return 2595.0 * std::log10(1.0 + f / 700.0); };
        auto mel2hz = [](double m) { return 700.0 * (std::pow(10.0, m / 2595.0) - 1.0); };
        const double fmx = fmax > 0 ? fmax : sr / 2.0;
        std::vector<double> mel_f(n_mels + 2);
        const double m0 = hz2mel(fmin), m1 = hz2mel(fmx);
        for (int i = 0; i < n_mels + 2; ++i) mel_f[i] = mel2hz(m0 + (m1 - m0) * i / (n_mels + 1));
        std::vector<float> wt((size_t)n_mels * FP, 0.f);
        for (int i = 0; i < n_mels; ++i) {
            const double enorm = 2.0 / (mel_f[i + 2] - mel_f[i]);
            for (int f = 0; f < F; ++f) {
                const double freq = (sr / 2.0) * f / (F - 1);
                const double lower = (freq - mel_f[i]) / (mel_f[i + 1] - mel_f[i]);
                const double upper = (mel_f[i + 2] - freq) / (mel_f[i + 2] - mel_f[i + 1]);
                const double v = std::max(0.0, std::min(lower, upper));
                wt[(size_t)i * FP + f] = (float)(v * enorm);
            }
        }
        HIPCHK(h, hipStreamSynchronize(h->stream));
        if (a.mel_wt) hipFree(a.mel_wt);
        a.mel_wt = nullptr;
        HIPCHK(h, hipMalloc(&a.mel_wt, wt.size() * sizeof(float)));
        HIPCHK(h, hipMemcpy(a.mel_wt, wt.data(), wt.size() * sizeof(float), hipMemcpyHostToDevice));
        a.sr = sr; a.n_fft = n_fft; a.n_mels = n_mels; a.fmin = fmin; a.fmax = fmax;
    }
    WS(h, "an.lin_tf", float, (size_t)B * n_frames * FP, lin_tf);
    WS(h, "an.mel_tf", float, (size_t)B * n_frames * n_mels, mel_tf);
    HIPCHK(h, launch_mag_ft_to_tf(h->stream, lin, lin_tf, B, F, n_frames, FP));
    int rc = run_single(h, dense_group(lin_tf, FP, a.mel_wt, nullptr, mel_tf, n_mels, B * n_frames, n_mels, FP, ACT_NONE));
    if (rc) return rc;
    HIPCHK(h, launch_tf_to_ft(h->stream, mel_tf, mel, B, n_mels, n_frames, n_mels));
    return TTS_OK;
}


int tts_db_convert(tts_handle_t h, const float* in, size_t n, int mode, float ref_db, float max_db, float* out) {
    DeviceScope dev_scope(h);
    if (!h || !in || !out || mode < 0 || mode > 3) return fail(h, TTS_ERR_INVALID, "db_convert: bad arguments");
    if (n == 0) return TTS_OK;
    if (mode == 1) {
        int* flag = nullptr;
        int rc = denorm_flag_arm(h, &flag);
        if (rc) return rc;
        HIPCHK(h, launch_any_below(h->stream, in, n, -100.0f, flag));
        if ((rc = denorm_flag_read(h))) return rc;
    }
    HIPCHK(h, launch_db_convert(h->stream, in, out, n, mode, ref_db, max_db));
    return TTS_OK;
}


int tts_debug_gl_plan(int T, int B, int win_length, int hop_length, int n_workers, int* items, int max_items, int* ring_frames) {
    if (T < 1 || B < 1 || win_length < 2 || win_length > TTS_GL_NFFT || hop_length < 1 || n_workers < 1 || !items || max_items < 0)
        return TTS_ERR_INVALID;
    const int ring = gl_stream_ring_frames(win_length, hop_length);
    if ((win_length + hop_length - 1) / hop_length > 8 || ring < 1) return TTS_ERR_UNSUPPORTED;
    int n_stage = 3;
    while (n_stage > 1 && gl_stream_ring_frames(win_length, hop_length, n_stage) <= 0) --n_stage;
    std::vector<int4> v;
    int slots = 0;
    const int n = gl_plan_items(T, B, win_length, hop_length, n_workers, n_stage, 0, 0, &v, &slots);
    if (ring_frames) *ring_frames = ring;
    for (int k = 0; k < n && k < max_items; ++k) {
        items[4 * k] = v[k].x; items[4 * k + 1] = v[k].y; items[4 * k + 2] = v[k].z; items[4 * k + 3] = v[k].w;
    }
    return n;
}


int tts_debug_gl_plan_ragged(const int32_t* n_frames, int B, int win_length, int hop_length, int n_workers, int* items, int max_items,
                             int* ring_frames) {
    if (!n_frames || B < 1 || win_length < 2 || win_length > TTS_GL_NFFT || hop_length < 1 || n_workers < 1 || !items || max_items < 0)
        return TTS_ERR_INVALID;
    int T_max = 0;
    for (int b = 0; b < B; ++b) {
        if (n_frames[b] < 1) return TTS_ERR_INVALID;
        T_max = std::max(T_max, (int)n_frames[b]);
    }
    const int ring = gl_stream_ring_frames(win_length, hop_length);
    if ((win_length + hop_length - 1) / hop_length > 8 || ring < 1) return TTS_ERR_UNSUPPORTED;
    int n_stage = 3;
    while (n_stage > 1 && gl_stream_ring_frames(win_length, hop_length, n_stage) <= 0) --n_stage;
    std::vector<int4> v;
    int slots = 0;
    const int n = gl_plan_items_ragged(n_frames, T_max, B, win_length, hop_length, n_workers, n_stage, 0, 0, &v, &slots);
    if (ring_frames) *ring_frames = ring;
    for (int k = 0; k < n && k < max_items; ++k) {
        items[4 * k] = v[k].x; items[4 * k + 1] = v[k].y; items[4 * k + 2] = v[k].z; items[4 * k + 3] = v[k].w;
    }
    return n;
}


int tts_debug_gemm(tts_handle_t h, const float* A, const float* Wt, float* C, int M, int N, int Cin, int ktaps, int T,
                   int pool) {
    DeviceScope dev_scope(h);
    if (!h || !A || !Wt || !C || M < 1 || N < 1 || Cin < 4 || (Cin & 3) || ktaps < 1 || T < 1 || M % T) return TTS_ERR_INVALID;
    GemmGroup g = conv_group(A, Cin, ktaps, T, Wt, nullptr, nullptr, nullptr, C, N, 0, M, N, ACT_NONE, pool);
    ProfScope ps(h, ST_DEBUG_GEMM, 1);
    const int slices = gemm_splitk_slices(g.K);
    if (slices > 1) {
        WS(h, "debug.splitk", float, (size_t)slices * M * N, part);
        HIPCHK(h, launch_gemm_splitk(h->stream, g, slices, part));
        return TTS_OK;
    }
    return run_single(h, g);
}


int tts_debug_hold(tts_handle_t h, int n_wgs, int lds_kb, double ms) {
    DeviceScope dev_scope(h);
    if (!h || n_wgs < 1 || lds_kb < 1 || lds_kb > 160) return TTS_ERR_INVALID;
    if (!h->debug_hooks) return fail(h, TTS_ERR_INVALID, "tts_debug_hold: a diagnostic; set the option \"debug_hooks\" to 1 on this handle first");
    static hipStream_t dbg = nullptr;
    static int* never = nullptr;
    static std::mutex dbg_mutex;
    std::lock_guard<std::mutex> lock(dbg_mutex);
    if (!dbg) {
        HIPCHK(h, hipStreamCreateWithFlags(&dbg, hipStreamNonBlocking));
        HIPCHK(h, hipMalloc(reinterpret_cast<void**>(&never), sizeof(int)));
        HIPCHK(h, hipMemset(never, 0, sizeof(int)));
    }
    HIPCHK(h, cu_hold_configure());
    HIPCHK(h, launch_cu_hold(dbg, n_wgs, never, ms, lds_kb));
    return TTS_OK;
}

}
```

### single-speaker-tts_amd/csrc/griffin_lim.h

```cpp
#pragma once
#include "tts_common.h"
#include <vector>

namespace tts {

#define TTS_GL_FP 1056
#define TTS_GL_NFFT 2048

struct GlParams {
    const float* mag;
    const float2* phase_in;
    float2* phase_out;
    float* wav;
    float* mse_partial;
    float* peak_partial;
    const float* window;
    const float* wlane;
    const float* rwss;
    const float2* tw1024;
    const float2* tw2048;
    const float2* tables;
    int T, FP, win, hop;
    int B;
    int ncol;
    const int4* items;
    int n_items, slots_per_utt;
    int n_workers;
    int ring_frames;
    int n_stage;
    int seeded, F;
    unsigned long long seed;
    unsigned* work_counter;
    unsigned* clear_counter;
    float2* mom_c;
    float mom_alpha;
    int mom_first;
    const int* n_frames;
    const float* rw_edge;
    int rw_E;
};

inline int gl_rw_edge_len(int n_fft, int win, int hop) { return n_fft + ((win + hop - 1) / hop - 1) * hop; }

void gl_build_wlane(const float* window, const float* rwss, int win, int hop, int T, float* out);
int gl_stream_ring_frames(int win, int hop, int n_stage = 1);
bool gl_stream_instantiated(int win, int hop);
hipError_t gl_plan_stream(GlParams& p, int n_workers, int n_stage = 1, int force_runs = 0, int force_run_len = 0, hipStream_t stream = nullptr);
int gl_plan_items(int T, int B, int win, int hop, int n_workers, int n_stage, int force_runs, int force_run_len,
                  std::vector<int4>* items, int* slots_per_utt, int* workers_out = nullptr);
int gl_plan_items_ragged(const int* lens, int T, int B, int win, int hop, int n_workers, int n_stage, int force_runs, int force_run_len,
                         std::vector<int4>* items, int* slots_per_utt, int* workers_out = nullptr);
hipError_t launch_gl_stream(hipStream_t s, const GlParams& p, int n_cus, int final_istft, int n_stage = 1);
hipError_t gl_configure();
size_t gl_state_bytes();
hipError_t launch_gl_mse_reduce(hipStream_t s, const float* partial, int B, int nchunks, float denom, float* mse);
hipError_t launch_gl_mse_reduce_ragged(hipStream_t s, const float* partial, int B, int nchunks, int F, const int* n_frames, int per_frame,
                                       float* mse);
hipError_t launch_mag_ft_to_tf(hipStream_t s, const float* in, float* out, int B, int F, int T, int FP, const int* n_frames = nullptr);
hipError_t launch_tf_to_ft(hipStream_t s, const float* in, float* out, int B, int F, int T, int FP);
hipError_t launch_phase_init(hipStream_t s, const float* init_ft, uint64_t seed, void* out, int B, int F, int T, int FP, const int* n_frames = nullptr);
hipError_t launch_denorm_power(hipStream_t s, const float* lin, float* mag, size_t rows, int F, int FP,
                               float ref_db, float max_db, float power, int* below_flag);
hipError_t launch_peak_normalize(hipStream_t s, float* wav, int B, int n);
hipError_t launch_peak_scale(hipStream_t s, float* wav, int B, int n, const float* partial, int nparts);
hipError_t launch_stft(hipStream_t s, const float* wav, int B, int n, int Tf, const float* window, int win, int hop,
                       const float2* tw1024, const float2* tw2048, float2* out, int FP);
hipError_t launch_cplx_tf_to_ft(hipStream_t s, const float2* in, float* out, int B, int F, int T, int FP, int mode,
                                float power);
hipError_t launch_db_convert(hipStream_t s, const float* in, float* out, size_t n, int mode, float ref_db, float max_db);
hipError_t launch_any_below(hipStream_t s, const float* in, size_t n, float lim, int* flag);

bool glg_supports(int n_fft);
hipError_t glg_configure();
hipError_t launch_glg_phase_init(hipStream_t s, const float* init_ft, uint64_t seed, float2* out, int B, int F, int T, int Fp, const int* n_frames = nullptr);
hipError_t launch_glg_istft(hipStream_t s, const float* mag, const float2* ph, const float* window, const float* rwss, const float2* tw,
                            float* frames, float* wav, int B, int T, int Fp, int n_fft, int win, int hop, const int* n_frames = nullptr);
hipError_t launch_glg_stft(hipStream_t s, const float* wav, int n, const float* window, const float2* tw, float2* out, int B, int Tf, int Fp,
                           int n_fft, int win, int hop, int mode, const float* mag, float* mse_partial, float2* mom_c = nullptr,
                           float mom_alpha = 0.f, int mom_first = 0, const int* n_frames = nullptr);

}
```

### single-speaker-tts_amd/csrc/griffin_lim.hip

```cpp
#include "tts_common.h"
#include "griffin_lim.h"
#include "fft_wave.h"
#include <algorithm>
#include <cmath>
#include <mutex>
#include <cstdlib>

namespace tts {


__device__ __forceinline__ void lds_barrier() {
    asm volatile("s_waitcnt lgkmcnt(0)\n\ts_barrier" ::: "memory");
}

typedef __attribute__((address_space(3))) int gl_lds_int;
__device__ __forceinline__ int gl_flag_load(int* p) {
    return __hip_atomic_load((gl_lds_int*)p, __ATOMIC_RELAXED, __HIP_MEMORY_SCOPE_WORKGROUP);
}
__device__ __forceinline__ void gl_flag_store(int* p, int v) {
    __hip_atomic_store((gl_lds_int*)p, v, __ATOMIC_RELAXED, __HIP_MEMORY_SCOPE_WORKGROUP);
}

__device__ __forceinline__ void mirror_bins(const cf (&z)[16], cf (&m)[16], cf* ex, int lane, cf nyq) {
    cf* wr = ex + lane;
    const cf* rd = ex + (1024 - lane);
#pragma unroll
    for (int c = 0; c < 16; ++c) wr[64 * c] = z[c];
    if (lane == 0) ex[1024] = nyq;
    wave_lds_sync();
#pragma unroll
    for (int c = 0; c < 16; ++c) m[c] = rd[-64 * c];
    wave_lds_sync();
}

#define GL_BIN(lane, j) ((j) < 8 ? (lane) + 64 * (j) : MH - (lane) - 64 * ((j) - 8))
#define GL_ROW(LO, HI, j) ((j) < 8 ? (LO)[64 * (j)] : (HI)[-64 * ((j) - 8)])
#define GL_NW 8
#define GL_THREADS 512
#define NFFT 2048
#define MH 1024

__device__ __forceinline__ float gl_stream_load(const float* p) { return __builtin_nontemporal_load(p); }
__device__ __forceinline__ void gl_stream_store(cf* p, cf v) { __builtin_nontemporal_store(v, p); }
#define GL_STREAM_LOAD(ptr) gl_stream_load(ptr)
#define GL_STREAM_STORE(ptr, val) gl_stream_store((ptr), (val))
__device__ __forceinline__ cf gl_seed_phasor(unsigned long long seed, unsigned long long idx) {
    unsigned x = (unsigned)idx ^ ((unsigned)(idx >> 32) * 0x9E3779B9u) ^ (unsigned)seed ^ ((unsigned)(seed >> 32) * 0x85EBCA6Bu);
    x ^= x >> 16; x *= 0x7FEB352Du; x ^= x >> 15; x *= 0x846CA68Bu; x ^= x >> 16;
    const float u = (float)(x >> 8) * (1.0f / 16777216.0f);
    return cmk(__builtin_amdgcn_cosf(u), __builtin_amdgcn_sinf(u));
}
__device__ __forceinline__ unsigned gl_pack_phasor(cf x) {
    const float den = fmaxf(fabsf(x.x) + fabsf(x.y), 1.0e-30f);
    const float p = x.y * __builtin_amdgcn_rcpf(den);
    return (__float_as_uint(p) & ~1u) | (__float_as_uint(x.x) >> 31);
}
__device__ __forceinline__ cf gl_unpack_phasor(unsigned c, float mag) {
    const float p = __uint_as_float(c);
    const float q = 1.0f - fabsf(p);
    const float xs = __uint_as_float(__float_as_uint(q) | (c << 31));
    const float g = mag * __builtin_amdgcn_rsqf(fmaf(p, p, q * q));
    return cmk(xs, p) * g;
}

__device__ __forceinline__ cf gl_normalise(cf x, float mag) {
    const float xr = x.x + 1.0e-17f;
    const float s2 = fmaf(xr, xr, fmaf(x.y, x.y, 1.0e-38f));
    const float g = mag * __builtin_amdgcn_rsqf(s2);
    return cmk(xr, x.y) * g;
}
typedef unsigned gl_state_t;
__device__ __forceinline__ gl_state_t gl_state_encode(cf x) { return gl_pack_phasor(x); }
__device__ __forceinline__ cf gl_state_decode(gl_state_t s, float mag) { return gl_unpack_phasor(s, mag); }
size_t gl_state_bytes() { return sizeof(gl_state_t); }

#define GL_NO_ITEM 0x7FFFFFFEu
enum { CT_OLA = 0, CT_SNEXT = 1, CT_OLB = 2 , CT_SWORDS = 16 };

template <int MODE, int WIN_CT, int HOP_CT, bool MSE, int NST = 1, bool SEEDED = false, bool MOM = false, bool RAG = false>
__global__ __launch_bounds__(GL_THREADS) void gl_stream_kernel(GlParams p) {
    static_assert(!SEEDED || MODE == 0, "the seeded start is an iteration's");
    static_assert(!MOM || (MODE == 0 && NST == 1), "momentum: one iteration per launch");
    static_assert(NST == 1 || (NST >= 2 && NST <= 3 && MODE == 0 && !MSE), "several iterations per launch: plain iterations only");
    extern __shared__ __attribute__((aligned(16))) unsigned char smem_raw[];
    const int win = WIN_CT ? WIN_CT : p.win;
    const int hop = HOP_CT ? HOP_CT : p.hop;
    const int ncol = (WIN_CT && HOP_CT) ? (WIN_CT + HOP_CT - 1) / (HOP_CT ? HOP_CT : 1) : p.ncol;
    const int halo = ncol - 1;
    const int wpad = (NFFT - win) >> 1;
    const int c_lo = wpad >> 7;
    const int c_hi = (wpad + win - 1) >> 7;
    constexpr int fz_lo_ = WIN_CT ? ((NFFT - WIN_CT) >> 1) >> 7 : 0;
    constexpr int fz_hi_ = WIN_CT ? (((NFFT - WIN_CT) >> 1) + WIN_CT - 1) >> 7 : 15;
    constexpr bool fz_ok_ = fz_lo_ <= 4 && fz_hi_ >= 11 && fz_hi_ <= 15;
    constexpr int FZ_LO = fz_ok_ ? fz_lo_ : 0, FZ_HI = fz_ok_ ? fz_hi_ : 15;
    const int n_sl = c_hi - c_lo + 1;
    const int S = 128 * n_sl;
    const int fs = 128 * c_lo;
    const int acc_len = S - hop;
    const int lag = (halo + 1) * hop > 2 * (MH - wpad) ? halo : halo + 1;
    const int R = p.ring_frames;
    const int ring_len = hop * R;
    const int ring_floats = (ring_len + acc_len + 128 + 3) & ~3;
    const int L = hop * (p.T - 1);
    int Tb_r = p.T;
    int L_r = L;
    const float* rw_head = nullptr;
    const float* rw_tail = nullptr;
#define GL_TB (RAG ? Tb_r : p.T)
#define GL_L (RAG ? L_r : L)
    cf* ex_all = reinterpret_cast<cf*>(smem_raw);
    int* ctrl = reinterpret_cast<int*>(ex_all + GL_NW * EX_CPLX);
    float* ringA = reinterpret_cast<float*>(ctrl + CT_SWORDS);

    const int tid = threadIdx.x;
    const int lane = tid & 63;
    const int wave = __builtin_amdgcn_readfirstlane(tid >> 6);
    cf* ex = ex_all + wave * EX_CPLX;

    if (tid == 0) ctrl[CT_SNEXT] = (int)atomicAdd(p.work_counter, 1u);
    if (tid == 0 && blockIdx.x == 0 && p.clear_counter) *p.clear_counter = 0u;
    cf twr[8];
#pragma unroll
    for (int j = 0; j < 8; ++j) twr[j] = reinterpret_cast<const cf*>(p.tw2048)[lane + 64 * j];
    FftTwReg tw;
#pragma unroll
    for (int k2 = 1; k2 < 16; ++k2) tw.a[k2 - 1] = reinterpret_cast<const cf*>(p.tables)[1024 + (k2 - 1) * 64 + lane];
#pragma unroll
    for (int d = 1; d < 4; ++d) tw.b[d - 1] = reinterpret_cast<const cf*>(p.tw1024)[16 * (lane & 15) * d];
    float wana[16][2], wsyn[16][2];
    {
        const float4* wa = reinterpret_cast<const float4*>(p.wlane + (0 * 64 + lane) * 32);
        const float4* ws = reinterpret_cast<const float4*>(p.wlane + (1 * 64 + lane) * 32);
#pragma unroll
        for (int q = 0; q < 8; ++q) {
            const float4 a4 = wa[q], s4 = ws[q];
            wana[2 * q][0] = a4.x; wana[2 * q][1] = a4.y; wana[2 * q + 1][0] = a4.z; wana[2 * q + 1][1] = a4.w;
            wsyn[2 * q][0] = s4.x; wsyn[2 * q][1] = s4.y; wsyn[2 * q + 1][0] = s4.z; wsyn[2 * q + 1][1] = s4.w;
        }
#pragma unroll
        for (int c = 0; c < 16; ++c)
            if (WIN_CT && (c < c_lo || c > c_hi)) { wana[c][0] = wana[c][1] = wsyn[c][0] = wsyn[c][1] = 0.f; }
#pragma unroll
        for (int c = 0; c < 16; ++c) wsyn[c][1] = -wsyn[c][1];
    }
    __syncthreads();
    int item = __builtin_amdgcn_readfirstlane(ctrl[CT_SNEXT]);

    auto decode_item = [&](int it, int& b, int& t0, int& len, int& slot, int& tb) {
        const int4 q = p.items[it];
        b = q.x; t0 = q.y; len = q.z; slot = q.w;
        if (RAG) tb = p.n_frames[q.x];
    };

    gl_state_t gc[16];
    float gs[16];
    gl_state_t nyq_c;
    float nyq_s;
    constexpr bool seeded = SEEDED;
#define GLS_LOAD_ROW(BASE_C, BASE_M, TF, TB)                                                    \
    {                                                                                           \
        int tf_ = (TF);                                                                         \
        tf_ = tf_ < 0 ? 0 : (tf_ >= (TB) ? (TB) - 1 : tf_);                                     \
        const gl_state_t* prow_ = (BASE_C) + (size_t)tf_ * p.FP;                                \
        const float* srow_ = (BASE_M) + (size_t)tf_ * p.FP;                                     \
        const gl_state_t* plo_ = prow_ + lane; const gl_state_t* phi_ = prow_ + (MH - lane);    \
        const float* slo_ = srow_ + lane; const float* shi_ = srow_ + (MH - lane);              \
        if (!seeded) {                                                                          \
            _Pragma("unroll") for (int j_ = 0; j_ < 16; ++j_) gc[j_] = GL_ROW(plo_, phi_, j_); \
            nyq_c = prow_[MH / 2];                                                              \
        }                                                                                       \
        _Pragma("unroll") for (int j_ = 0; j_ < 16; ++j_) gs[j_] = GL_STREAM_LOAD(j_ < 8 ? slo_ + 64 * j_ : shi_ - 64 * (j_ - 8)); \
        nyq_s = srow_[MH / 2];                                                                  \
    }
#define GLS_TOUCH_ROW()                                                                                              \
    asm volatile("" : "+v"(gc[0]), "+v"(gc[1]), "+v"(gc[2]), "+v"(gc[3]), "+v"(gc[4]), "+v"(gc[5]), "+v"(gc[6]),       \
                      "+v"(gc[7]), "+v"(gc[8]), "+v"(gc[9]), "+v"(gc[10]), "+v"(gc[11]), "+v"(gc[12]), "+v"(gc[13]), \
                      "+v"(gc[14]), "+v"(gc[15]), "+v"(nyq_c));                                                      \
    asm volatile("" : "+v"(gs[0]), "+v"(gs[1]), "+v"(gs[2]), "+v"(gs[3]), "+v"(gs[4]), "+v"(gs[5]), "+v"(gs[6]),       \
                      "+v"(gs[7]), "+v"(gs[8]), "+v"(gs[9]), "+v"(gs[10]), "+v"(gs[11]), "+v"(gs[12]), "+v"(gs[13]), \
                      "+v"(gs[14]), "+v"(gs[15]), "+v"(nyq_s));
    const gl_state_t* x_in = reinterpret_cast<const gl_state_t*>(p.phase_in);
    gl_state_t* x_out = reinterpret_cast<gl_state_t*>(p.phase_out);

#define GLS_URGENCY(NEXT_INDEX)                                                                    \
    {                                                                                              \
        const int d_ = __builtin_amdgcn_readfirstlane((NEXT_INDEX) - gl_flag_load(ctrl + CT_OLA)); \
        if (d_ <= 1) __builtin_amdgcn_s_setprio(3);                                                \
        else if (d_ <= 3) __builtin_amdgcn_s_setprio(2);                                           \
        else if (d_ <= 5) __builtin_amdgcn_s_setprio(1);                                           \
        else __builtin_amdgcn_s_setprio(0);                                                        \
    }

    auto split_pass = [&](cf (&gk)[16], cf mid, cf (&v)[16]) __attribute__((always_inline)) {
        cf* wr = ex + (MH - lane);
#pragma unroll
        for (int c = 0; c < 8; ++c) {
            cf xk = gk[c];
            cf xm = gk[8 + c];
            if (c == 0 && lane == 0) { xk.y = 0.f; xm.y = 0.f; }
            const cf e = cadd_conj(xk, xm);
            const cf o = cmul_conj(csub_conj(xk, xm), twr[c]);
            v[c] = cconj_add_pi(e, o);
            wr[-64 * c] = cadd_mi(e, o);
        }
        if (lane == 0) ex[MH / 2] = cscale(mid, 2.0f);
        wave_lds_sync();
#pragma unroll
        for (int j = 8; j < 16; ++j) v[j] = ex[lane + 64 * j];
        wave_lds_sync();
    };
    auto synth_window = [&](int t, cf (&v)[16]) __attribute__((always_inline)) {
        if (t >= halo && t + halo < GL_TB) {
#pragma unroll
            for (int c = 0; c < 16; ++c) v[c] = v[c] * cmk(wsyn[c][0], wsyn[c][1]);
        } else {
            const float* rwp = (RAG ? (t < halo ? rw_head : rw_tail) : p.rwss) + (size_t)t * hop + wpad;
#pragma unroll
            for (int c0 = 0; c0 < 16; c0 += 4) {
#pragma unroll
                for (int c = c0; c < c0 + 4; ++c) {
                    const int nw0 = 2 * (lane + 64 * c) - wpad;
                    const bool i0 = nw0 >= 0 && nw0 < win, i1 = nw0 + 1 >= 0 && nw0 + 1 < win;
                    const float r0 = rwp[i0 ? nw0 : 0], r1 = rwp[i1 ? nw0 + 1 : 0];
                    v[c] = cmk(i0 ? v[c].x * wana[c][0] * r0 : 0.f, i1 ? -v[c].y * wana[c][1] * r1 : 0.f);
                }
                asm volatile("" ::: "memory");
            }
        }
    };
    float pk = 0.f;
    auto overlap_add = [&](float* ring, int chain, int idx, int s, int t, int b, int run_t0, int run_len, const cf (&v)[16])
                           __attribute__((always_inline)) {
        float* const lds_f = reinterpret_cast<float*>(smem_raw);
        const int e_wr = (int)(ring - lds_f) + hop * s + 2 * lane;
        const int e_rd = e_wr + (s == 0 ? ring_len : 0);
        int wo[8], ro[8];
#pragma unroll
        for (int k = 0; k < 8; ++k) {
            wo[k] = e_wr + 256 * k;
            ro[k] = e_rd + 256 * k;
            if (2 * k < n_sl) asm volatile("" : "+v"(wo[k]), "+v"(ro[k]));
        }
        const int qb_edge = 128 * ((acc_len - 1) >> 7);
        unsigned keep0 = qb_edge + 2 * lane < acc_len ? ~0u : 0u, keep1 = qb_edge + 2 * lane + 1 < acc_len ? ~0u : 0u;
        asm volatile("" : "+v"(keep0), "+v"(keep1));
        while (gl_flag_load(ctrl + chain) < idx) __builtin_amdgcn_s_sleep(1);
        asm volatile("" ::: "memory");
        cf fin[16];
        {
            cf o[16];
#pragma unroll
            for (int c = 0; c < 16; ++c) {
                const int j = c - c_lo;
                o[c] = cmk(0.f, 0.f);
                if (j < 0 || j >= n_sl) continue;
                const int qb = 128 * j;
                const float* rp = lds_f + ro[j >> 1] + 128 * (j & 1);
                if (qb < acc_len) o[c] = cmk(rp[0], rp[1]);
            }
            asm volatile("" ::: "memory");
#pragma unroll
            for (int c = 0; c < 16; ++c) {
                const int j = c - c_lo;
                if (j < 0 || j >= n_sl) continue;
                const int qb = 128 * j;
                cf a = v[c];
                if (qb < acc_len) {
                    cf acc = o[c];
                    if (qb + 127 >= acc_len) {
                        acc.x = __uint_as_float(__float_as_uint(acc.x) & keep0);
                        acc.y = __uint_as_float(__float_as_uint(acc.y) & keep1);
                    }
                    a = cadd(acc, v[c]);
                }
                float* wp = lds_f + wo[j >> 1] + 128 * (j & 1);
                wp[0] = a.x;
                wp[1] = a.y;
                if (MODE == 1) fin[c] = a;
            }
        }
        asm volatile("" ::: "memory");
        if (lane == 0) gl_flag_store(ctrl + chain, idx + 1);
        if (MODE == 1) {
            asm volatile("" ::: "memory");
            const int q_fin = wpad - fs;
            const int y0 = t * hop + fs - MH;
            const bool emit = (t >= run_t0 || run_t0 == 0) && (t < run_t0 + run_len || run_t0 + run_len == GL_TB);
            float* wb = p.wav + (size_t)b * L;
#pragma unroll
            for (int c = 0; c < 16; ++c) {
                const int j = c - c_lo;
                if (j < 0 || j >= n_sl) continue;
                const int qb = 128 * j;
                if (qb + 127 >= q_fin && qb < q_fin + hop) {
                    const int q = qb + 2 * lane;
                    const int y = y0 + q;
                    const cf a = fin[c];
                    if (emit && q >= q_fin && q < q_fin + hop && y >= 0 && y < GL_L) { wb[y] = a.x; pk = fmaxf(pk, fabsf(a.x)); }
                    if (emit && q + 1 >= q_fin && q + 1 < q_fin + hop && y + 1 >= 0 && y + 1 < GL_L) { wb[y + 1] = a.y; pk = fmaxf(pk, fabsf(a.y)); }
                }
            }
        }
    };
    auto fft_input = [&](const float* ring, int idx, int sm, int tm, int y_base, cf (&v)[16]) __attribute__((always_inline)) {
        const int ylo = tm * hop + wpad - MH;
        const bool edge = ylo < 0 || ylo + win > GL_L;
        if (!edge && (hop * sm + S <= ring_len || R - sm > lag)) {
            const float* const lds_f = reinterpret_cast<const float*>(smem_raw);
            const int e_rd = (int)(ring - lds_f) + hop * sm + 2 * lane;
            int ro[8];
#pragma unroll
            for (int k = 0; k < 8; ++k) {
                ro[k] = e_rd + 256 * k;
                if (2 * k < n_sl) asm("" : "+v"(ro[k]));
            }
#pragma unroll
            for (int c = 0; c < 16; ++c) {
                const int j = c - c_lo;
                if (j < 0 || j >= n_sl) { v[c] = cmk(0.f, 0.f); continue; }
                const float* sf = lds_f + ro[j >> 1] + 128 * (j & 1);
                v[c] = cmk(wana[c][0], wana[c][1]) * cmk(sf[0], sf[1]);
            }
        } else {
            const int lap0 = (idx - lag) / R;
            const int ub = y_base + lap0 * ring_len;
#pragma unroll
            for (int c = 0; c < 16; ++c) {
                float x[2] = {0.f, 0.f};
#pragma unroll
                for (int e = 0; e < 2; ++e) {
                    const int f = 2 * (lane + 64 * c) + e;
                    const int nw = f - wpad;
                    if (nw >= 0 && nw < win) {
                        int y = ylo + nw;
                        y = y < 0 ? -y : y;
                        y = y >= GL_L ? 2 * (GL_L - 1) - y : y;
                        int off = y - ub, lap = lap0;
                        if (off >= ring_len) { off -= ring_len; ++lap; }
                        else if (off < 0) { off += ring_len; --lap; }
                        const int pos = (off < acc_len && lap * R > idx) ? ring_len + off : off;
                        x[e] = wana[c][e] * ring[pos];
                    }
                }
                v[c] = cmk(x[0], x[1]);
            }
        }
    };
    auto merge_pass = [&](const cf (&v)[16], auto&& sink) __attribute__((always_inline)) -> cf {
#pragma unroll
        for (int j = 8; j < 16; ++j) ex[lane + 64 * j] = v[j];
        if (lane == 0) ex[MH] = v[0];
        wave_lds_sync();
        cf zm[8];
        const cf* rd = ex + (MH - lane);
#pragma unroll
        for (int c = 0; c < 8; ++c) zm[c] = rd[-64 * c];
#pragma unroll
        for (int c = 0; c < 8; ++c) {
            const cf e = cadd_conj(v[c], zm[c]);
            const cf o = cmul(csub_conj(v[c], zm[c]), twr[c]);
            sink(c, cadd_mi(e, o));
            sink(8 + c, cconj_add_pi(e, o));
        }
        wave_lds_sync();
        return cscale(cconj(v[8]), 2.0f);
    };

    const int lead = NST * halo;
    bool have_row = false;
    while (item < p.n_items) {
        int b, run_t0, run_len, slot;
        decode_item(item, b, run_t0, run_len, slot, Tb_r);
        if (RAG) {
            L_r = hop * (Tb_r - 1);
            const int cut = NFFT + L_r - p.rw_E;
            rw_head = p.rw_edge + (size_t)b * 2 * p.rw_E;
            rw_tail = rw_head + p.rw_E - (cut > 0 ? cut : 0);
        }
        const float* magb = p.mag + (size_t)b * p.T * p.FP;
        const gl_state_t* phb = x_in + (size_t)b * p.T * p.FP;
        const int n_idx = run_len + NST * (halo + lag);
        const bool late = n_idx >= 4 * GL_NW;
        const int i_res = n_idx - 3 * GL_NW;
        unsigned next_item_reg = GL_NO_ITEM;
        if (tid == 0 && !late) next_item_reg = atomicAdd(p.work_counter, 1u);
        if (!have_row) GLS_LOAD_ROW(phb, magb, run_t0 - lead + wave, GL_TB)
        have_row = false;
        for (int q = tid; q < acc_len + 128; q += GL_THREADS) {
#pragma unroll
            for (int k = 0; k < NST; ++k) ringA[k * ring_floats + ring_len + q] = 0.f;
        }
        if (tid == 0) { ctrl[CT_OLA] = 0; ctrl[CT_OLB] = 0; ctrl[CT_OLB + 1] = 0; ctrl[CT_SNEXT] = (int)next_item_reg; }
        __syncthreads();
        int next_item = __builtin_amdgcn_readfirstlane(ctrl[CT_SNEXT]);
        int nb = b, nt0 = 0, nlen = 0, nslot = 0, nTb = p.T;
        if (!late && next_item < p.n_items) decode_item(next_item, nb, nt0, nlen, nslot, nTb);

        const int y_base_a = (run_t0 - lead) * hop - MH + fs;
        float mse_acc = 0.f;
        pk = 0.f;
        int s = wave % R;
        GLS_TOUCH_ROW()
        for (int i = wave; i < n_idx; i += GL_NW) {
            const int t = run_t0 - lead + i;
            const bool valid = t >= 0 && t < GL_TB;
            unsigned drawn = 0;
            if (late && i == i_res && lane == 0) drawn = atomicAdd(p.work_counter, 1u);
            if (late && i + GL_NW >= n_idx) {
                int nv;
                while ((nv = gl_flag_load(ctrl + CT_SNEXT)) == (int)GL_NO_ITEM) __builtin_amdgcn_s_sleep(1);
                next_item = __builtin_amdgcn_readfirstlane(nv);
                if (next_item < p.n_items) decode_item(next_item, nb, nt0, nlen, nslot, nTb);
            }
            GLS_URGENCY(i)
            cf v[16];
            if (valid) {
                cf gk[16];
                if (seeded) {
                    const unsigned long long row0 = (unsigned long long)b * p.F * p.T + (unsigned long long)t;
#pragma unroll
                    for (int j = 0; j < 16; ++j) {
                        const cf e = gl_seed_phasor(p.seed, row0 + (unsigned long long)GL_BIN(lane, j) * p.T);
                        gk[j] = cmk(gs[j] * e.x, gs[j] * e.y);
                    }
                    const cf en = gl_seed_phasor(p.seed, row0 + (unsigned long long)(MH / 2) * p.T);
                    split_pass(gk, cmk(nyq_s * en.x, nyq_s * en.y), v);
                } else {
#pragma unroll
                    for (int j = 0; j < 16; ++j) gk[j] = gl_state_decode(gc[j], gs[j]);
                    split_pass(gk, gl_state_decode(nyq_c, nyq_s), v);
                }
            } else {
#pragma unroll
                for (int j = 0; j < 16; ++j) asm volatile("v_mov_b64 %0, 0" : "=v"(v[j]));
            }
            GLS_URGENCY(i)
#define GLS_NEXT_ROW()                                                                                                   \
            if (i + GL_NW < n_idx) {                                                                                     \
                GLS_LOAD_ROW(phb, magb, t + GL_NW, GL_TB)                                                                \
            } else if (next_item < p.n_items) {                                                                          \
                GLS_LOAD_ROW(x_in + (size_t)nb * p.T * p.FP, p.mag + (size_t)nb * p.T * p.FP, nt0 - lead + wave, (RAG ? nTb : p.T)) \
                have_row = true;                                                                                         \
            }
            if (NST == 1) {
                GLS_NEXT_ROW()
            }
            if (valid) {
                fft1024(v, ex, tw, lane);
                synth_window(t, v);
            }
            if (late && i == i_res && lane == 0) gl_flag_store(ctrl + CT_SNEXT, (int)drawn);
            overlap_add(ringA, CT_OLA, i, s, t, b, run_t0, run_len, v);
            if (NST == 1) {
                GLS_TOUCH_ROW()
            }
            GLS_URGENCY(i + GL_NW)

            int sk = s, ik = i, tk = t;
            float* ring_k = ringA;
            int yb_k = y_base_a;
#pragma nounroll
            for (int k = 1; k < NST; ++k) {
                const int i_prev = ik, s_prev = sk;
                const float* ring_prev = ring_k;
                const int yb_prev = yb_k;
                ik -= halo + lag;
                tk -= lag;
                sk -= halo + lag;
                sk += sk < 0 ? R : 0;
                ring_k += ring_floats;
                yb_k += halo * hop;
                const bool valid_k = ik >= 0 && tk >= 0 && tk < GL_TB;
                {
                    const int tq = tk < 0 ? 0 : (tk >= GL_TB ? GL_TB - 1 : tk);
                    const float* mrow_ = magb + (size_t)tq * p.FP;
                    const float* mlo_ = mrow_ + lane; const float* mhi_ = mrow_ + (MH - lane);
#pragma unroll
                    for (int j = 0; j < 16; ++j) gs[j] = GL_ROW(mlo_, mhi_, j);
                    nyq_s = mrow_[MH / 2];
                }
                if (valid_k) {
                    int sm = s_prev - lag;
                    sm += sm < 0 ? R : 0;
                    fft_input(ring_prev, i_prev, sm, tk, yb_prev, v);
                    fft1024<FZ_LO, FZ_HI>(v, ex, tw, lane);
                    cf gk[16];
                    const cf xmid = merge_pass(v, [&](int c, cf x) { gk[c] = gl_normalise(x, gs[c]); });
                    split_pass(gk, gl_normalise(xmid, nyq_s), v);
                } else {
#pragma unroll
                    for (int j = 0; j < 16; ++j) asm volatile("v_mov_b64 %0, 0" : "=v"(v[j]));
                }
                if (k + 1 == NST) {
                    GLS_NEXT_ROW()
                }
                if (ik >= 0) {
                    if (valid_k) {
                        fft1024(v, ex, tw, lane);
                        synth_window(tk, v);
                    }
                    overlap_add(ring_k, CT_OLB + k - 1, ik, sk, tk, b, run_t0, run_len, v);
                }
            }
            if (NST > 1) GLS_TOUCH_ROW()
            const int jj = ik, sb = sk;
            if (MODE == 0 && jj >= halo + lag && jj < halo + lag + run_len) {
                const int tm = tk - lag;
                int sm = sb - lag;
                sm += sm < 0 ? R : 0;
                const float* mrow = magb + (size_t)tm * p.FP;
                float mg[16];
                if (MSE) {
#pragma unroll
                    for (int c = 0; c < 16; ++c) mg[c] = fabsf(GL_STREAM_LOAD(c < 8 ? mrow + lane + 64 * c : mrow + (MH - lane) - 64 * (c - 8)));
                }
                cf cp[16], cp_mid = cmk(0.f, 0.f);
                cf* const crow = MOM ? reinterpret_cast<cf*>(p.mom_c) + ((size_t)b * p.T + tm) * p.FP : nullptr;
                cf* const clo = MOM ? crow + lane : nullptr;
                cf* const chi = MOM ? crow + (MH - lane) : nullptr;
                const bool mom_prev = MOM && !p.mom_first;
                if (MOM) {
#pragma unroll
                    for (int c = 0; c < 16; ++c) cp[c] = cmk(0.f, 0.f);
                    if (mom_prev) {
#pragma unroll
                        for (int c = 0; c < 16; ++c) cp[c] = __builtin_nontemporal_load(c < 8 ? clo + 64 * c : chi - 64 * (c - 8));
                        cp_mid = crow[MH / 2];
                    }
                }
                auto mom_t = [&](cf x, cf prev) __attribute__((always_inline)) -> cf {
                    return mom_prev ? cadd(x, cscale(csub(x, prev), p.mom_alpha)) : x;
                };
                fft_input(ring_k, jj, sm, tm, yb_k, v);
                fft1024<FZ_LO, FZ_HI>(v, ex, tw, lane);
                GLS_URGENCY(i + GL_NW)
                if (MOM && MSE) mse_acc = 0.f;
                gl_state_t* orow = x_out + ((size_t)b * p.T + tm) * p.FP;
                gl_state_t* olo = orow + lane;
                gl_state_t* ohi = orow + (MH - lane);
                const cf xmid = merge_pass(v, [&](int c, cf x) {
                    if (MOM) {
                        GL_STREAM_STORE(c < 8 ? clo + 64 * c : chi - 64 * (c - 8), x);
                        __builtin_nontemporal_store(gl_state_encode(mom_t(x, cp[c])), c < 8 ? olo + 64 * c : ohi - 64 * (c - 8));
                    } else
                    __builtin_nontemporal_store(gl_state_encode(x), c < 8 ? olo + 64 * c : ohi - 64 * (c - 8));
                    if (MSE) {
                        const float d = mg[c] - (float)MH * sqrtf(fmaf(x.x, x.x, x.y * x.y));
                        mse_acc += d * d;
                    }
                });
                if (lane == 0) {
                    if (MOM) crow[MH / 2] = xmid;
                    __builtin_nontemporal_store(gl_state_encode(MOM ? mom_t(xmid, cp_mid) : xmid), orow + MH / 2);
                    if (MSE) {
                        const float d = fabsf(mrow[MH / 2]) - (float)MH * sqrtf(fmaf(xmid.x, xmid.x, xmid.y * xmid.y));
                        mse_acc += d * d;
                    }
                }
                if (MOM && MSE) {
                    float r = mse_acc;
#pragma unroll
                    for (int o = 32; o > 0; o >>= 1) r += __shfl_xor(r, o);
                    if (lane == 0) p.mse_partial[(size_t)b * p.T + tm] = r;
                }
            }
            s += GL_NW;
            s -= s >= R ? R : 0;
        }
        __builtin_amdgcn_s_setprio(0);
        if ((MODE == 0 && MSE && !MOM) || (MODE == 1 && p.peak_partial)) {
            float r = MODE == 0 ? mse_acc : pk;
#pragma unroll
            for (int o = 32; o > 0; o >>= 1) r = MODE == 0 ? r + __shfl_xor(r, o) : fmaxf(r, __shfl_xor(r, o));
            __syncthreads();
            float* red = reinterpret_cast<float*>(ex_all);
            if (lane == 0) red[wave] = r;
            __syncthreads();
            if (tid == 0) {
                float a = 0.f;
                for (int w = 0; w < GL_NW; ++w) a = MODE == 0 ? a + red[w] : fmaxf(a, red[w]);
                float* part = (MODE == 0 ? p.mse_partial : p.peak_partial) + (size_t)b * p.slots_per_utt + (slot & 0xffff);
                part[0] = a;
                for (int q = 1; q <= (slot >> 16); ++q) part[q] = 0.f;
            }
        }
        __syncthreads();
        item = next_item;
    }
#undef GLS_LOAD_ROW
#undef GL_TB
#undef GL_L
#undef GLS_NEXT_ROW
#undef GLS_TOUCH_ROW
#undef GLS_URGENCY
}


namespace {
struct GlStreamGeom { int c_lo, n_sl, S, acc_len, halo; };
GlStreamGeom gl_stream_geom(int win, int hop) {
    GlStreamGeom g;
    const int wpad = (NFFT - win) >> 1;
    g.c_lo = wpad >> 7;
    g.n_sl = ((wpad + win - 1) >> 7) - g.c_lo + 1;
    g.S = 128 * g.n_sl;
    g.acc_len = g.S - hop;
    g.halo = (win + hop - 1) / hop - 1;
    return g;
}
}

int gl_stream_ring_frames(int win, int hop, int n_stage) {
    const GlStreamGeom g = gl_stream_geom(win, hop);
    if (g.acc_len < 0) return 0;
    const int wpad = (NFFT - win) >> 1;
    const int lag = (g.halo + 1) * hop > 2 * (MH - wpad) ? g.halo : g.halo + 1;
    const int budget = (160 * 1024 - (int)(GL_NW * EX_CPLX * sizeof(cf)) - CT_SWORDS * (int)sizeof(int)) / (int)sizeof(float) / n_stage - g.acc_len - 132;
    int need = 9 + lag + (g.S + hop - 1) / hop + 1;
    const int reach = (g.S + win + 2 * hop + hop - 1) / hop;
    need = std::max(need, std::max(reach, GL_NW));
    const int R = std::min(budget / hop, std::max(64, need));
    return R >= need ? R : 0;
}

size_t gl_stream_lds_bytes(const GlParams& p) {
    const GlStreamGeom g = gl_stream_geom(p.win, p.hop);
    return (size_t)(GL_NW * EX_CPLX) * sizeof(cf) + CT_SWORDS * sizeof(int) +
           (size_t)(p.n_stage < 1 ? 1 : p.n_stage) * (size_t)((p.hop * p.ring_frames + g.acc_len + 128 + 3) & ~3) * sizeof(float);
}

namespace {
struct GlRun { int b, t0, len; };
struct GlCutCost { double interior, edge; };
GlCutCost gl_cut_cost(int halo, int lag, int n_stage) {
    const double c = (halo + lag) * n_stage / 4.0;
    return GlCutCost{c * (5.5 / 6.0), c * 0.5};
}
bool gl_deal(const int* lens, int T, int B, int W, double M, const GlCutCost& cc, int min_len_all, std::vector<std::vector<GlRun>>& workers, double* makespan) {
    workers.assign((size_t)W, {});
    int b = 0, t = 0, w = 0;
    double load = 0.0, worst = 0.0;
    while (b < B) {
        if (w >= W) return false;
        const int Tb = lens ? lens[b] : T;
        const int min_len = std::min(Tb, min_len_all);
        const int rest = Tb - t;
        const double left = t > 0 ? cc.interior : cc.edge;
        const double whole = rest + left + cc.edge;
        if (load + whole <= M + 1e-9) {
            workers[w].push_back(GlRun{b, t, rest});
            load += whole;
            ++b; t = 0;
            continue;
        }
        int len = (int)std::floor(M - load - left - cc.interior + 1e-9);
        if (rest - len < min_len) len = rest - min_len;
        if (len >= min_len) {
            workers[w].push_back(GlRun{b, t, len});
            load += len + left + cc.interior;
            t += len;
        } else if (workers[w].empty()) {
            return false;
        }
        worst = std::max(worst, load);
        ++w; load = 0.0;
    }
    worst = std::max(worst, load);
    if (makespan) *makespan = worst;
    return true;
}
}

int gl_plan_items(int T, int B, int win, int hop, int n_workers, int n_stage, int force_runs, int force_run_len,
                  std::vector<int4>* items, int* slots_per_utt, int* workers_out) {
    return gl_plan_items_ragged(nullptr, T, B, win, hop, n_workers, n_stage, force_runs, force_run_len, items, slots_per_utt, workers_out);
}

int gl_plan_items_ragged(const int* lens, int T, int B, int win, int hop, int n_workers, int n_stage, int force_runs, int force_run_len,
                         std::vector<int4>* items, int* slots_per_utt, int* workers_out) {
    auto len_of = [&](int b) { return lens ? lens[b] : T; };
    long long total_frames = 0;
    int T_min = len_of(0), T_top = len_of(0);
    for (int b = 0; b < B; ++b) {
        total_frames += len_of(b);
        T_min = std::min(T_min, len_of(b));
        T_top = std::max(T_top, len_of(b));
    }
    if (lens && T_min == T_top) {
        lens = nullptr;
        T = T_top;
    }
    const int ncol = (win + hop - 1) / hop, halo = ncol - 1;
    n_stage = n_stage < 1 ? 1 : (n_stage > 3 ? 3 : n_stage);
    n_workers = n_workers < 1 ? 1 : n_workers;
    const int wpad = (TTS_GL_NFFT - win) >> 1;
    const int lag = (halo + 1) * hop > 2 * (TTS_GL_NFFT / 2 - wpad) ? halo : halo + 1;
    std::vector<std::vector<GlRun>> workers;
    int forced_len = 0;
    if (force_runs >= 1 && force_runs <= T_top) forced_len = ((T_top + force_runs - 1) / force_runs + GL_NW - 1) / GL_NW * GL_NW;
    if (force_run_len >= GL_NW) forced_len = force_run_len / GL_NW * GL_NW;
    if (forced_len > 0) {
        for (int t0 = 0; t0 < T_top; t0 += forced_len)
            for (int b = 0; b < B; ++b)
                if (t0 < len_of(b)) workers.push_back({GlRun{b, t0, std::min(forced_len, len_of(b) - t0)}});
    } else {
        const GlCutCost cc = gl_cut_cost(halo, lag, n_stage);
        const long long per_worker = total_frames / n_workers;
        const int min_len_all = (int)std::max<long long>(GL_NW / 2, std::min<long long>(GL_NW, per_worker));
        const int min_len = std::min(T_min, min_len_all);
        const double total = (double)total_frames + (double)B * 2 * cc.edge;
        double lo = std::max(total / n_workers, (double)min_len + 2 * cc.edge), best_t = 1e300;
        std::vector<std::vector<GlRun>> cand;
        int best_step = -1;
        for (int step = 0; step < 400; ++step) {
            const double M = lo * (1.0 + 0.0025 * step);
            double t = 0.0;
            if (!gl_deal(lens, T, B, n_workers, M, cc, min_len_all, cand, &t)) continue;
            if (t < best_t - 1e-9) { best_t = t; workers = cand; best_step = step; }
        }
        if (lens && best_step > 0) {
            for (int sub = 1; sub < 16; ++sub) {
                const double M = lo * (1.0 + 0.0025 * (best_step - 1 + sub / 16.0));
                double t = 0.0;
                if (!gl_deal(lens, T, B, n_workers, M, cc, min_len_all, cand, &t)) continue;
                if (t < best_t - 1e-9) { best_t = t; workers = cand; }
            }
        }
        if (workers.empty()) {
            for (int b = 0; b < B; ++b) workers.push_back({GlRun{b, 0, len_of(b)}});
        }
    }
    std::vector<int> slot_of((size_t)B, 0), runs_of((size_t)B, 0);
    for (const auto& w : workers) for (const GlRun& r : w) ++runs_of[r.b];
    int spu = 1;
    for (int b = 0; b < B; ++b) spu = std::max(spu, runs_of[b]);
    std::vector<int> slot_at;
    auto slot_word = [&](const GlRun& r) {
        int ord = 0;
        for (const auto& w : workers) for (const GlRun& q : w) if (q.b == r.b && q.t0 < r.t0) ++ord;
        const int pad = ord == runs_of[r.b] - 1 ? spu - runs_of[r.b] : 0;
        return ord | (pad << 16);
    };
    items->clear();
    size_t depth = 0;
    for (const auto& w : workers) depth = std::max(depth, w.size());
    if (lens) {
        std::vector<std::pair<double, const GlRun*>> rest;
        for (const auto& w : workers) {
            double before = 0.0;
            for (size_t d = 0; d < w.size(); ++d) {
                if (d == 0) items->push_back(make_int4(w[d].b, w[d].t0, w[d].len, slot_word(w[d])));
                else rest.push_back({before, &w[d]});
                before += w[d].len + 11.0;
            }
        }
        std::stable_sort(rest.begin(), rest.end(), [](const std::pair<double, const GlRun*>& a, const std::pair<double, const GlRun*>& b) { return a.first < b.first; });
        for (const auto& e : rest) items->push_back(make_int4(e.second->b, e.second->t0, e.second->len, slot_word(*e.second)));
        depth = 0;
    }
    for (size_t d = 0; d < depth; ++d) {
        std::vector<std::pair<double, const GlRun*>> level;
        for (const auto& w : workers) {
            if (w.size() <= d) continue;
            double before = 0.0;
            for (size_t q = 0; q < d; ++q) before += w[q].len;
            level.push_back({before, &w[d]});
        }
        std::stable_sort(level.begin(), level.end(), [](const std::pair<double, const GlRun*>& a, const std::pair<double, const GlRun*>& b) { return a.first < b.first; });
        for (const auto& e : level) items->push_back(make_int4(e.second->b, e.second->t0, e.second->len, slot_word(*e.second)));
    }
    if (workers_out) {
        int nw = 0;
        for (const auto& w : workers) nw += !w.empty();
        *workers_out = nw;
    }
    if (slots_per_utt) *slots_per_utt = spu;
    return (int)items->size();
}

hipError_t gl_plan_stream(GlParams& p, int n_workers, int n_stage, int force_runs, int force_run_len, hipStream_t stream) {
    struct Table { int4* ptr = nullptr; hipEvent_t ready = nullptr; hipStream_t owner = nullptr; bool seen = false; };
    struct Plan { std::vector<int4> items; int slots = 1, workers = 1; std::map<int, Table> dev; };
    struct Pool { char* base = nullptr; size_t used = 0, size = 0; };
    static std::map<std::vector<int>, Plan> cache;
    static std::map<int, Pool> pools;
    static std::mutex cache_mutex;
    std::lock_guard<std::mutex> lock(cache_mutex);
    p.ring_frames = gl_stream_ring_frames(p.win, p.hop, 1);
    const std::vector<int> key = {p.T, p.B, p.win, p.hop, n_workers, n_stage, force_runs, force_run_len};
    Plan& plan = cache[key];
    if (plan.items.empty())
        gl_plan_items(p.T, p.B, p.win, p.hop, n_workers, n_stage, force_runs, force_run_len, &plan.items, &plan.slots, &plan.workers);
    int dev = 0;
    hipError_t e = hipGetDevice(&dev);
    if (e != hipSuccess) return e;
    Table& t = plan.dev[dev];
    if (!t.ptr) {
        const size_t bytes = (plan.items.size() * sizeof(int4) + 255) & ~(size_t)255;
        Pool& pool = pools[dev];
        if (pool.used + bytes > pool.size) {
            const size_t block = std::max<size_t>(bytes, 1u << 20);
            void* m = nullptr;
            if ((e = hipMalloc(&m, block)) != hipSuccess) return e;
            pool.base = static_cast<char*>(m); pool.used = 0; pool.size = block;
        }
        int4* d = reinterpret_cast<int4*>(pool.base + pool.used);
        hipEvent_t ev = nullptr;
        if ((e = hipEventCreateWithFlags(&ev, hipEventDisableTiming)) != hipSuccess) return e;
        if ((e = hipMemcpyAsync(d, plan.items.data(), plan.items.size() * sizeof(int4), hipMemcpyHostToDevice, stream)) != hipSuccess ||
            (e = hipEventRecord(ev, stream)) != hipSuccess) {
            (void)hipEventDestroy(ev);
            return e;
        }
        pool.used += bytes;
        t.ptr = d; t.ready = ev; t.owner = stream; t.seen = false;
    } else if (!t.seen) {
        if (hipEventQuery(t.ready) == hipSuccess) t.seen = true;
        else if (stream != t.owner && (e = hipStreamWaitEvent(stream, t.ready, 0)) != hipSuccess) return e;
    }
    p.items = t.ptr;
    p.n_items = (int)plan.items.size();
    p.slots_per_utt = plan.slots;
    p.n_workers = plan.workers;
    return hipSuccess;
}

template <int MODE, int W, int H, bool MSE, int NST = 1, bool RAG = false>
static hipError_t gl_stream_set_attr() {
    hipError_t e = hipFuncSetAttribute(reinterpret_cast<const void*>(&gl_stream_kernel<MODE, W, H, MSE, NST, false, false, RAG>),
                                       hipFuncAttributeMaxDynamicSharedMemorySize, 160 * 1024);
    if (e != hipSuccess || MODE != 0) return e;
    return hipFuncSetAttribute(reinterpret_cast<const void*>(&gl_stream_kernel<0, W, H, MSE, NST, true, false, RAG>),
                               hipFuncAttributeMaxDynamicSharedMemorySize, 160 * 1024);
}
template <int W, int H, bool MSE, bool SEEDED, bool RAG = false>
static hipError_t gl_stream_set_attr_mom() {
    return hipFuncSetAttribute(reinterpret_cast<const void*>(&gl_stream_kernel<0, W, H, MSE, 1, SEEDED, true, RAG>),
                               hipFuncAttributeMaxDynamicSharedMemorySize, 160 * 1024);
}

bool gl_stream_instantiated(int win, int hop) { return (win == 1102 && hop == 275) || (win == 800 && hop == 200); }

template <int W, int H, bool RAG>
static hipError_t gl_stream_launch_wh(hipStream_t s, const GlParams& p, dim3 grid, size_t lds, int final_istft, int n_stage, bool mse) {
#define GLS_LAUNCH_N(MODE, M, N)                                                                                         \
    {                                                                                                                    \
        if (MODE == 0 && p.seeded) hipLaunchKernelGGL((gl_stream_kernel<0, W, H, M, N, true, false, RAG>), grid, dim3(GL_THREADS), lds, s, p);   \
        else hipLaunchKernelGGL((gl_stream_kernel<MODE, W, H, M, N, false, false, RAG>), grid, dim3(GL_THREADS), lds, s, p);        \
    }
    if (p.mom_c && !final_istft) {
        if (mse && p.seeded) return hipErrorInvalidValue;
        if (mse) hipLaunchKernelGGL((gl_stream_kernel<0, W, H, true, 1, false, true, RAG>), grid, dim3(GL_THREADS), lds, s, p);
        else if (p.seeded) hipLaunchKernelGGL((gl_stream_kernel<0, W, H, false, 1, true, true, RAG>), grid, dim3(GL_THREADS), lds, s, p);
        else hipLaunchKernelGGL((gl_stream_kernel<0, W, H, false, 1, false, true, RAG>), grid, dim3(GL_THREADS), lds, s, p);
        return hipGetLastError();
    }
    if (n_stage == 3) GLS_LAUNCH_N(0, false, 3)
    else if (n_stage == 2) GLS_LAUNCH_N(0, false, 2)
    else if (final_istft) GLS_LAUNCH_N(1, false, 1)
    else if (mse) GLS_LAUNCH_N(0, true, 1)
    else GLS_LAUNCH_N(0, false, 1)
#undef GLS_LAUNCH_N
    return hipGetLastError();
}

hipError_t launch_gl_stream(hipStream_t s, const GlParams& p_in, int n_cus, int final_istft, int n_stage) {
    GlParams p = p_in;
    p.n_stage = n_stage;
    p.ring_frames = gl_stream_ring_frames(p.win, p.hop, n_stage);
    if (p.ring_frames < GL_NW || n_stage < 1 || n_stage > 3 || (n_stage > 1 && (final_istft || p.mse_partial))) return hipErrorInvalidValue;
    if (p.mom_c && !final_istft && n_stage != 1) return hipErrorInvalidValue;
    const size_t lds = gl_stream_lds_bytes(p);
    const int nwg = p.n_workers > 0 && p.n_workers < n_cus ? p.n_workers : (p.n_items < n_cus ? p.n_items : n_cus);
    const dim3 grid(nwg);
    const bool mse = p.mse_partial != nullptr;
    if (p.n_frames) {
        if (!p.rw_edge || p.rw_E != gl_rw_edge_len(NFFT, p.win, p.hop)) return hipErrorInvalidValue;
        if (p.win == 1102 && p.hop == 275) return gl_stream_launch_wh<1102, 275, true>(s, p, grid, lds, final_istft, n_stage, mse);
        if (p.win == 800 && p.hop == 200) return gl_stream_launch_wh<800, 200, true>(s, p, grid, lds, final_istft, n_stage, mse);
        return hipErrorInvalidValue;
    }
    if (p.win == 1102 && p.hop == 275) return gl_stream_launch_wh<1102, 275, false>(s, p, grid, lds, final_istft, n_stage, mse);
    if (p.win == 800 && p.hop == 200) return gl_stream_launch_wh<800, 200, false>(s, p, grid, lds, final_istft, n_stage, mse);
    return hipErrorInvalidValue;
}

template <int W, int H, bool RAG>
static hipError_t gl_stream_configure_wh() {
    hipError_t e;
    if ((e = gl_stream_set_attr<0, W, H, true, 1, RAG>()) != hipSuccess) return e;
    if ((e = gl_stream_set_attr<0, W, H, false, 1, RAG>()) != hipSuccess) return e;
    if ((e = gl_stream_set_attr<0, W, H, false, 2, RAG>()) != hipSuccess) return e;
    if ((e = gl_stream_set_attr<0, W, H, false, 3, RAG>()) != hipSuccess) return e;
    if ((e = gl_stream_set_attr<1, W, H, false, 1, RAG>()) != hipSuccess) return e;
    if ((e = gl_stream_set_attr_mom<W, H, false, false, RAG>()) != hipSuccess) return e;
    if ((e = gl_stream_set_attr_mom<W, H, false, true, RAG>()) != hipSuccess) return e;
    if ((e = gl_stream_set_attr_mom<W, H, true, false, RAG>()) != hipSuccess) return e;
    return hipSuccess;
}
hipError_t gl_stream_configure() {
    hipError_t e = gl_stream_configure_wh<1102, 275, false>();
    if (e == hipSuccess) e = gl_stream_configure_wh<800, 200, false>();
    if (e == hipSuccess) e = gl_stream_configure_wh<1102, 275, true>();
    if (e == hipSuccess) e = gl_stream_configure_wh<800, 200, true>();
    return e;
}

void gl_build_wlane(const float* window, const float* rwss, int win, int hop, int T, float* out) {
    const int wpad = (NFFT - win) / 2;
    const int halo = (win + hop - 1) / hop - 1;
    const int t_ref = halo < T ? halo : T - 1;
    for (int c = 0; c < 16; ++c)
        for (int e = 0; e < 2; ++e)
            for (int lane = 0; lane < 64; ++lane) {
                const int nw = 2 * (lane + 64 * c) + e - wpad;
                const bool in = nw >= 0 && nw < win;
                const float w = in ? window[nw] * (0.5f / (float)MH) : 0.f;
                const float rw = in ? rwss[(size_t)t_ref * hop + wpad + nw] : 0.f;
                out[(0 * 64 + lane) * 32 + 2 * c + e] = w;
                out[(1 * 64 + lane) * 32 + 2 * c + e] = w * rw;
            }
}

static hipError_t stft_configure();

hipError_t gl_configure() {
    const hipError_t e = gl_stream_configure();
    return e != hipSuccess ? e : stft_configure();
}

__global__ __launch_bounds__(GL_THREADS) void stft_kernel(const float* __restrict__ wav, int n, int Tf,
                                                          const float* __restrict__ window, int win, int hop,
                                                          const cf* __restrict__ tw1024, const cf* __restrict__ tw2048,
                                                          cf* __restrict__ out, int FP) {
    extern __shared__ __attribute__((aligned(16))) unsigned char smem_raw[];
    cf* ex_all = reinterpret_cast<cf*>(smem_raw);
    cf* twR = ex_all + GL_NW * EX_CPLX;
    cf* twA = twR + 1024;
    float* wtab = reinterpret_cast<float*>(twA + 15 * 64);
    const int tid = threadIdx.x, lane = tid & 63, wave = tid >> 6;
    cf* ex = ex_all + wave * EX_CPLX;
    for (int i = tid; i < win; i += GL_THREADS) wtab[i] = window[i];
    for (int i = tid; i < 1024; i += GL_THREADS) twR[i] = tw2048[i];
    for (int i = tid; i < 15 * 64; i += GL_THREADS) twA[i] = tw1024[(i & 63) * ((i >> 6) + 1)];
    FftTw tw;
#pragma unroll
    for (int d = 1; d < 4; ++d) tw.b[d - 1] = tw1024[16 * (lane & 15) * d];
    tw.a = twA + lane;
    __syncthreads();
    const int b = blockIdx.y;
    const int t = blockIdx.x * GL_NW + wave;
    if (t >= Tf) return;
    const float* y = wav + (size_t)b * n;
    const int wpad = (NFFT - win) >> 1;
    const int ylo = t * hop + wpad - MH;
    cf v[16];
#pragma unroll
    for (int j = 0; j < 16; ++j) {
        const int nn = 2 * (lane + 64 * j);
        float x[2] = {0.f, 0.f};
#pragma unroll
        for (int e = 0; e < 2; ++e) {
            const int nw = nn + e - wpad;
            if (nw >= 0 && nw < win) {
                int yi = ylo + nw;
                yi = yi < 0 ? -yi : yi;
                yi = yi >= n ? 2 * (n - 1) - yi : yi;
                x[e] = wtab[nw] * y[yi];
            }
        }
        v[j] = cmk(x[0], x[1]);
    }
    fft1024(v, ex, tw, lane);
#pragma unroll
    for (int c = 0; c < 16; ++c) ex[lane + 64 * c] = v[c];
    wave_lds_sync();
    cf* orow = out + ((size_t)b * Tf + t) * FP;
#pragma unroll
    for (int c = 0; c < 16; ++c) {
        const int k = lane + 64 * c;
        const cf zk = v[c];
        const cf zr = ex[(MH - k) & (MH - 1)];
        const cf e = cscale(cadd_conj(zk, zr), 0.5f);
        const cf o = cmul(cscale(csub_conj(zk, zr), 0.5f), twR[k]);
        orow[k] = cadd_mi(e, o);
    }
    if (lane == 0) orow[MH] = cmk(v[0].x - v[0].y, 0.f);
    if (lane < FP - MH - 1) orow[MH + 1 + lane] = cmk(0.f, 0.f);
}

static hipError_t stft_configure() {
    return hipFuncSetAttribute(reinterpret_cast<const void*>(&stft_kernel), hipFuncAttributeMaxDynamicSharedMemorySize,
                               160 * 1024);
}

hipError_t launch_stft(hipStream_t s, const float* wav, int B, int n, int Tf, const float* window, int win, int hop,
                       const float2* tw1024, const float2* tw2048, float2* out, int FP) {
    const size_t lds = (size_t)(GL_NW * EX_CPLX + 1024 + 15 * 64) * sizeof(cf) + (size_t)((win + 3) & ~3) * sizeof(float);
    dim3 grid((Tf + GL_NW - 1) / GL_NW, B);
    hipLaunchKernelGGL(stft_kernel, grid, dim3(GL_THREADS), lds, s, wav, n, Tf, window, win, hop,
                       reinterpret_cast<const cf*>(tw1024), reinterpret_cast<const cf*>(tw2048), reinterpret_cast<cf*>(out), FP);
    return hipGetLastError();
}

__global__ void cplx_tf_to_ft_kernel(const cf* in, float* out, int F, int T, int FP, int mode, float power) {
    __shared__ cf tile[32][33];
    const int b = blockIdx.z;
    const int f0 = blockIdx.y * 32, t0 = blockIdx.x * 32;
    const int tx = threadIdx.x, ty = threadIdx.y;
    for (int i = ty; i < 32; i += 8) {
        const int t = t0 + i, f = f0 + tx;
        tile[i][tx] = (t < T && f < F) ? in[((size_t)b * T + t) * FP + f] : cmk(0.f, 0.f);
    }
    __syncthreads();
    for (int i = ty; i < 32; i += 8) {
        const int f = f0 + i, t = t0 + tx;
        if (f < F && t < T) {
            const cf z = tile[tx][i];
            const size_t o = ((size_t)b * F + f) * T + t;
            if (mode == 0) {
                reinterpret_cast<cf*>(out)[o] = z;
            } else {
                const float m = sqrtf(z.x * z.x + z.y * z.y);
                out[o] = power == 1.0f ? m : (power == 2.0f ? m * m : powf(m, power));
            }
        }
    }
}
hipError_t launch_cplx_tf_to_ft(hipStream_t s, const float2* in, float* out, int B, int F, int T, int FP, int mode,
                                float power) {
    dim3 grid((T + 31) / 32, (F + 31) / 32, B);
    hipLaunchKernelGGL(cplx_tf_to_ft_kernel, grid, dim3(32, 8), 0, s, reinterpret_cast<const cf*>(in), out, F, T, FP, mode, power);
    return hipGetLastError();
}

__global__ void db_convert_kernel(const float* in, float* out, size_t n, int mode, float ref_db, float max_db) {
    const float range = fabsf(ref_db) + fabsf(max_db);
    for (size_t i = (size_t)blockIdx.x * blockDim.x + threadIdx.x; i < n; i += (size_t)gridDim.x * blockDim.x) {
        const float x = in[i];
        float y;
        if (mode == 0) y = (float)(20.0 * log10((double)(x != x ? x : fmaxf(1e-5f, x))));
        else if (mode == 1) y = exp2f(x * (0.05f * 3.3219280948873623f));
// ... 193 lines not shown
```

Measured before the change: 4.393 million.

## Chain Griffin-Lim rounds in one launch with per-span neighbour flags

Several Griffin-Lim rounds now run inside a single persistent launch. Work items from later rounds wait on per-item completion counters covering only their overlapping neighbour runs, instead of a full kernel boundary between rounds. This removes launch gaps and grid-wide barriers between iterations, so late items of one round can overlap early items of the next. In exchange it adds spin-waiting and release/acquire fences, a timeout fallback that marks results invalid, extra span metadata in the plan table, and debug hooks.

Result: slower. 4.325 million (-1.5%).

```diff
diff --git a/include/sstts_hip.h b/include/sstts_hip.h
--- a/include/sstts_hip.h
+++ b/include/sstts_hip.h
@@ -163,6 +163,9 @@
 int tts_decoder_kernel_choice(tts_handle_t h, int B, int T_sent, int pipelined);
 int tts_debug_workspace(tts_handle_t h, const char* name, void** dptr, size_t* bytes);
 int tts_debug_gl_plan(int T, int B, int win_length, int hop_length, int n_workers, int* items, int max_items, int* ring_frames);
+int tts_debug_gl_chain_plan(int T, int B, int win_length, int hop_length, int n_workers, int n_stage, int run_len, int* items,
+                            int* spans, int max_items);
+long long tts_debug_gl_chain_rounds(tts_handle_t h);
 int tts_debug_gl_plan_ragged(const int32_t* n_frames, int B, int win_length, int hop_length, int n_workers,
                              int* items, int max_items, int* ring_frames);
 int tts_debug_gemm(tts_handle_t h, const float* A, const float* Wt, float* C, int M, int N, int Cin, int ktaps, int T,
diff --git a/single-speaker-tts_amd/_hip.py b/single-speaker-tts_amd/_hip.py
--- a/single-speaker-tts_amd/_hip.py
+++ b/single-speaker-tts_amd/_hip.py
@@ -113,6 +113,8 @@
     'tts_debug_hold': (c_int, [c_void_p, c_int, c_int, ctypes.c_double]),
     'tts_debug_gemm': (c_int, [c_void_p, c_void_p, c_void_p, c_void_p, c_int, c_int, c_int, c_int, c_int, c_int]),
     'tts_debug_gl_plan': (c_int, [c_int, c_int, c_int, c_int, c_int, POINTER(c_int), c_int, POINTER(c_int)]),
+    'tts_debug_gl_chain_plan': (c_int, [c_int, c_int, c_int, c_int, c_int, c_int, c_int, POINTER(c_int), POINTER(c_int), c_int]),
+    'tts_debug_gl_chain_rounds': (ctypes.c_longlong, [c_void_p]),
     'tts_debug_gl_plan_ragged': (c_int, [POINTER(c_int32), c_int, c_int, c_int, c_int, POINTER(c_int), c_int, POINTER(c_int)]),
     'tts_device_info': (c_int, [c_void_p, c_char_p, POINTER(c_int)]),
 }
diff --git a/single-speaker-tts_amd/csrc/api_handle.hip b/single-speaker-tts_amd/csrc/api_handle.hip
--- a/single-speaker-tts_amd/csrc/api_handle.hip
+++ b/single-speaker-tts_amd/csrc/api_handle.hip
@@ -355,6 +355,19 @@
         if (status) HIPCHK(h, hipMemset(h->pd_sync + 64 * h->pd_clusters + 1, 0, sizeof(int)));
         if (status) h->persistent_decoder = 0;
         if (status) return pd_timed_out(h);
+    }
+    if (h->gl_chain_used) {
+        h->gl_chain_used = false;
+        int status = 0;
+        HIPCHK(h, hipMemcpy(&status, h->gl_chain_words, sizeof(int), hipMemcpyDeviceToHost));
+        if (status) {
+            HIPCHK(h, hipMemset(h->gl_chain_words, 0, sizeof(int)));
+            h->gl_chain = 0;
+            return fail(h, TTS_ERR_HIP,
+                        "griffin_lim: a run of a chained launch waited for its neighbours longer than the bound; the waveforms of "
+                        "that call are invalid -- the handle has switched to one launch per round "
+                        "(tts_set_option(h, \"gl_chain\", 1) switches back)");
+        }
     }
     return TTS_OK;
 }
@@ -681,6 +694,7 @@
         h->persistent_decoder = value;
     }
     else if (!std::strcmp(key, "gl_pair")) h->gl_pair = value;
+    else if (!std::strcmp(key, "gl_chain")) h->gl_chain = value != 0;
     else if (!std::strcmp(key, "gl_momentum")) {
         if (value < 0 || value > 999) return fail(h, TTS_ERR_INVALID, "gl_momentum: thousandths of the momentum, 0 .. 999");
         h->gl_momentum = value;
@@ -700,7 +714,8 @@
     }
     else if (!std::strcmp(key, "debug_hooks")) h->debug_hooks = value;
     else if (!std::strcmp(key, "pd_debug_delay") || !std::strcmp(key, "gl_runs") || !std::strcmp(key, "gl_run_len") ||
-             !std::strcmp(key, "timeline") || !std::strcmp(key, "gl_workers") || !std::strcmp(key, "pd_rows")) {
+             !std::strcmp(key, "timeline") || !std::strcmp(key, "gl_workers") || !std::strcmp(key, "pd_rows") ||
+             !std::strcmp(key, "gl_chain_delay") || !std::strcmp(key, "gl_chain_delay_wg")) {
         if (!h->debug_hooks && value != 0)
             return fail(h, TTS_ERR_INVALID, std::string(key) + ": a test hook; set the option \"debug_hooks\" to 1 on this handle first");
         if (!std::strcmp(key, "pd_debug_delay")) h->pd_debug_delay = value;
@@ -708,6 +723,8 @@
         else if (!std::strcmp(key, "gl_run_len")) h->gl_run_len = value;
         else if (!std::strcmp(key, "gl_workers")) h->gl_workers = value;
         else if (!std::strcmp(key, "pd_rows")) h->pd_rows = value;
+        else if (!std::strcmp(key, "gl_chain_delay")) h->gl_chain_delay = value < 0 ? 0 : (value > 4096 ? 4096 : value);
+        else if (!std::strcmp(key, "gl_chain_delay_wg")) h->gl_chain_delay_wg = value;
         else h->timeline = value;
     }
     else if (!std::strcmp(key, "reserve_cus")) {
diff --git a/single-speaker-tts_amd/csrc/api_internal.h b/single-speaker-tts_amd/csrc/api_internal.h
--- a/single-speaker-tts_amd/csrc/api_internal.h
+++ b/single-speaker-tts_amd/csrc/api_internal.h
@@ -206,6 +206,12 @@
     int gl_pair = 3;
     int gl_momentum = 0;
     int gl_wide = -1;
+    int gl_chain = 1;
+    unsigned* gl_chain_words = nullptr;
+    unsigned gl_chain_base = 0;
+    hipStream_t gl_chain_stream = nullptr;
+    bool gl_chain_used = false;
+    long long gl_chain_rounds = 0;
     int n_cus_dev = 0;
     bool pd_configured = false;
     int debug_hooks = 0;
@@ -214,6 +220,8 @@
     int gl_run_len = 0;
     int timeline = 0;
     int gl_workers = 0;
+    int gl_chain_delay = 0;
+    int gl_chain_delay_wg = 0;
     unsigned* gl_ring = nullptr;
     unsigned gl_ring_seq = 0;
     unsigned* gl_ring_last = nullptr;
diff --git a/single-speaker-tts_amd/csrc/api_stages.hip b/single-speaker-tts_amd/csrc/api_stages.hip
--- a/single-speaker-tts_amd/csrc/api_stages.hip
+++ b/single-speaker-tts_amd/csrc/api_stages.hip
@@ -511,6 +511,19 @@
         q.work_counter = ring + (h->gl_ring_seq++ % GL_RING);
         h->gl_ring_last = q.work_counter;
     };
+    constexpr int GL_CHAIN_WORDS = 16384;
+    const bool chain_ok = h->gl_chain > 0 && !p.mom_c && !n_frames && std::max(p.n_items, pw.n_items) <= GL_CHAIN_WORDS;
+    unsigned* chain_words = nullptr;
+    if (chain_ok) {
+        WS(h, "gl.chain_done", unsigned, (size_t)4 + GL_CHAIN_WORDS, cw);
+        if (cw != h->gl_chain_words || h->gl_chain_stream != h->stream) {
+            HIPCHK(h, hipMemsetAsync(cw, 0, ((size_t)4 + GL_CHAIN_WORDS) * sizeof(unsigned), h->stream));
+            h->gl_chain_words = cw;
+            h->gl_chain_stream = h->stream;
+            h->gl_chain_base = 0;
+        }
+        chain_words = cw;
+    }
     const bool seed_in_kernel = !init_ft && n_iter >= 1;
     if (!phase_ready && !seed_in_kernel) HIPCHK(h, launch_phase_init(h->stream, init_ft, seed, ph0, B, F, T, FP, p.n_frames));
     p.F = pw.F = F;
@@ -533,6 +546,32 @@
             q.mom_first = it == 0;
             q.mse_partial = want_mse ? msep : nullptr;
             if (want_mse) mse_chunks = q.mom_c ? T : q.slots_per_utt;
+            int rounds = 1;
+            if (chain_ok && !q.seeded && !want_mse && n_stage == per_launch) {
+                for (;; ++rounds) {
+                    const int it2 = it + rounds * per_launch;
+                    if (n_iter - (mse ? 1 : 0) - it2 < per_launch) break;
+                    if ((two_cuts && launch_idx + rounds >= wide_from) != wide) break;
+                }
+            }
+            if (rounds >= 2) {
+                q.chain_rounds = rounds;
+                q.chain_done = chain_words + 4;
+                q.chain_status = reinterpret_cast<int*>(chain_words);
+                q.chain_base = h->gl_chain_base;
+                q.dbg_wg = h->debug_hooks ? h->gl_chain_delay_wg : 0;
+                q.dbg_delay = h->debug_hooks ? h->gl_chain_delay : 0;
+                h->gl_chain_base += (unsigned)rounds;
+                h->gl_chain_used = true;
+                h->gl_chain_rounds += rounds;
+                next_counter(q);
+                HIPCHK(h, launch_gl_stream_chain(h->stream, q, wide ? n_cus : free_cus, n_stage));
+                q.chain_rounds = 0;
+                if (rounds & 1) std::swap(cur, nxt);
+                it += rounds * n_stage;
+                launch_idx += rounds;
+                continue;
+            }
             next_counter(q);
             HIPCHK(h, launch_gl_stream(h->stream, q, wide ? n_cus : free_cus, 0, n_stage));
             std::swap(cur, nxt);
@@ -1183,6 +1222,27 @@
 }
 
 
+int tts_debug_gl_chain_plan(int T, int B, int win_length, int hop_length, int n_workers, int n_stage, int run_len, int* items, int* spans,
+                            int max_items) {
+    if (T < 1 || B < 1 || win_length < 2 || win_length > TTS_GL_NFFT || hop_length < 1 || n_workers < 1 || n_stage < 1 || n_stage > 3 ||
+        run_len < 0 || !items || !spans || max_items < 0)
+        return TTS_ERR_INVALID;
+    if ((win_length + hop_length - 1) / hop_length > 8 || gl_stream_ring_frames(win_length, hop_length, n_stage) < 1) return TTS_ERR_UNSUPPORTED;
+    std::vector<int4> v, sp;
+    int slots = 0;
+    const int n = gl_plan_items(T, B, win_length, hop_length, n_workers, n_stage, 0, run_len, &v, &slots);
+    gl_plan_spans(v, win_length, hop_length, n_stage, &sp);
+    for (int k = 0; k < n && k < max_items; ++k) {
+        items[4 * k] = v[k].x; items[4 * k + 1] = v[k].y; items[4 * k + 2] = v[k].z; items[4 * k + 3] = v[k].w;
+        spans[3 * k] = sp[k].x; spans[3 * k + 1] = sp[k].y; spans[3 * k + 2] = sp[k].z;
+    }
+    return n;
+}
+
+
+long long tts_debug_gl_chain_rounds(tts_handle_t h) { return h ? h->gl_chain_rounds : (long long)TTS_ERR_INVALID; }
+
+
 int tts_debug_gl_plan_ragged(const int32_t* n_frames, int B, int win_length, int hop_length, int n_workers, int* items, int max_items,
                              int* ring_frames) {
     if (!n_frames || B < 1 || win_length < 2 || win_length > TTS_GL_NFFT || hop_length < 1 || n_workers < 1 || !items || max_items < 0)
diff --git a/single-speaker-tts_amd/csrc/griffin_lim.h b/single-speaker-tts_amd/csrc/griffin_lim.h
--- a/single-speaker-tts_amd/csrc/griffin_lim.h
+++ b/single-speaker-tts_amd/csrc/griffin_lim.h
@@ -38,6 +38,12 @@
     const int* n_frames;
     const float* rw_edge;
     int rw_E;
+    int chain_rounds;
+    const int4* chain_span;
+    unsigned* chain_done;
+    unsigned chain_base;
+    int* chain_status;
+    int dbg_wg, dbg_delay;
 };
 
 inline int gl_rw_edge_len(int n_fft, int win, int hop) { return n_fft + ((win + hop - 1) / hop - 1) * hop; }
@@ -51,6 +57,8 @@
 int gl_plan_items_ragged(const int* lens, int T, int B, int win, int hop, int n_workers, int n_stage, int force_runs, int force_run_len,
                          std::vector<int4>* items, int* slots_per_utt, int* workers_out = nullptr);
 hipError_t launch_gl_stream(hipStream_t s, const GlParams& p, int n_cus, int final_istft, int n_stage = 1);
+hipError_t launch_gl_stream_chain(hipStream_t s, const GlParams& p, int n_cus, int n_stage);
+void gl_plan_spans(const std::vector<int4>& items, int win, int hop, int n_stage, std::vector<int4>* spans);
 hipError_t gl_configure();
 size_t gl_state_bytes();
 hipError_t launch_gl_mse_reduce(hipStream_t s, const float* partial, int B, int nchunks, float denom, float* mse);
diff --git a/single-speaker-tts_amd/csrc/griffin_lim.hip b/single-speaker-tts_amd/csrc/griffin_lim.hip
--- a/single-speaker-tts_amd/csrc/griffin_lim.hip
+++ b/single-speaker-tts_amd/csrc/griffin_lim.hip
@@ -75,11 +75,13 @@
 size_t gl_state_bytes() { return sizeof(gl_state_t); }
 
 #define GL_NO_ITEM 0x7FFFFFFEu
-enum { CT_OLA = 0, CT_SNEXT = 1, CT_OLB = 2 , CT_SWORDS = 16 };
-
-template <int MODE, int WIN_CT, int HOP_CT, bool MSE, int NST = 1, bool SEEDED = false, bool MOM = false, bool RAG = false>
+enum { CT_OLA = 0, CT_SNEXT = 1, CT_OLB = 2 , CT_DRAIN = 4 , CT_SWORDS = 16 };
+#define GL_CHAIN_SPIN_LIMIT 4000000u
+
+template <int MODE, int WIN_CT, int HOP_CT, bool MSE, int NST = 1, bool SEEDED = false, bool MOM = false, bool RAG = false, bool CHAIN = false>
 __global__ __launch_bounds__(GL_THREADS) void gl_stream_kernel(GlParams p) {
     static_assert(!SEEDED || MODE == 0, "the seeded start is an iteration's");
+    static_assert(!CHAIN || (MODE == 0 && !MSE && !SEEDED && !MOM && !RAG), "chained rounds: plain iterations of a uniform batch only");
     static_assert(!MOM || (MODE == 0 && NST == 1), "momentum: one iteration per launch");
     static_assert(NST == 1 || (NST >= 2 && NST <= 3 && MODE == 0 && !MSE), "several iterations per launch: plain iterations only");
     extern __shared__ __attribute__((aligned(16))) unsigned char smem_raw[];
@@ -119,6 +121,7 @@
     cf* ex = ex_all + wave * EX_CPLX;
 
     if (tid == 0) ctrl[CT_SNEXT] = (int)atomicAdd(p.work_counter, 1u);
+    if (CHAIN && tid == 0) ctrl[CT_DRAIN] = 0;
     if (tid == 0 && blockIdx.x == 0 && p.clear_counter) *p.clear_counter = 0u;
     cf twr[8];
 #pragma unroll
@@ -147,10 +150,22 @@
     __syncthreads();
     int item = __builtin_amdgcn_readfirstlane(ctrl[CT_SNEXT]);
 
+    const int n_total = CHAIN ? p.n_items * p.chain_rounds : p.n_items;
     auto decode_item = [&](int it, int& b, int& t0, int& len, int& slot, int& tb) {
-        const int4 q = p.items[it];
+        const int4 q = p.items[CHAIN ? it % p.n_items : it];
         b = q.x; t0 = q.y; len = q.z; slot = q.w;
         if (RAG) tb = p.n_frames[q.x];
+    };
+    auto decode_chain = [&](int it, int& round, int& pos, int& lo, int& hi) {
+        round = it / p.n_items;
+        const int4 q = p.chain_span[it - round * p.n_items];
+        pos = q.x; lo = q.y; hi = q.z;
+    };
+    auto span_ok = [&](int lo, int hi, unsigned want) -> bool {
+        bool ok = true;
+        for (int k = lo + lane; k <= hi; k += 64)
+            ok &= (int)(__hip_atomic_load(p.chain_done + k, __ATOMIC_RELAXED, __HIP_MEMORY_SCOPE_AGENT) - want) >= 0;
+        return __all(ok);
     };
 
     gl_state_t gc[16];
@@ -182,6 +197,8 @@
                       "+v"(gs[14]), "+v"(gs[15]), "+v"(nyq_s));
     const gl_state_t* x_in = reinterpret_cast<const gl_state_t*>(p.phase_in);
     gl_state_t* x_out = reinterpret_cast<gl_state_t*>(p.phase_out);
+#define GL_X_IN(ROUND) (CHAIN && ((ROUND) & 1) ? reinterpret_cast<const gl_state_t*>(p.phase_out) : x_in)
+#define GL_X_OUT(ROUND) (CHAIN && ((ROUND) & 1) ? const_cast<gl_state_t*>(x_in) : x_out)
 
 #define GLS_URGENCY(NEXT_INDEX)                                                                    \
     {                                                                                              \
@@ -369,9 +386,11 @@
 
     const int lead = NST * halo;
     bool have_row = false;
-    while (item < p.n_items) {
+    while (item < n_total) {
         int b, run_t0, run_len, slot;
         decode_item(item, b, run_t0, run_len, slot, Tb_r);
+        int round = 0, pos = 0, sp_lo = 0, sp_hi = -1;
+        if (CHAIN) decode_chain(item, round, pos, sp_lo, sp_hi);
         if (RAG) {
             L_r = hop * (Tb_r - 1);
             const int cut = NFFT + L_r - p.rw_E;
@@ -379,23 +398,53 @@
             rw_tail = rw_head + p.rw_E - (cut > 0 ? cut : 0);
         }
         const float* magb = p.mag + (size_t)b * p.T * p.FP;
-        const gl_state_t* phb = x_in + (size_t)b * p.T * p.FP;
+        const gl_state_t* phb = GL_X_IN(round) + (size_t)b * p.T * p.FP;
         const int n_idx = run_len + NST * (halo + lag);
         const bool late = n_idx >= 4 * GL_NW;
         const int i_res = n_idx - 3 * GL_NW;
         unsigned next_item_reg = GL_NO_ITEM;
-        if (tid == 0 && !late) next_item_reg = atomicAdd(p.work_counter, 1u);
+        if (!CHAIN && tid == 0 && !late) next_item_reg = atomicAdd(p.work_counter, 1u);
+        if (CHAIN) {
+            if (wave == 0 && round > 0) {
+                const unsigned want = p.chain_base + (unsigned)round;
+                unsigned spins = 0;
+                while (!span_ok(sp_lo, sp_hi, want)) {
+                    __builtin_amdgcn_s_sleep(8);
+                    if ((++spins & 255u) == 0 &&
+                        (spins > GL_CHAIN_SPIN_LIMIT || __hip_atomic_load(p.chain_status, __ATOMIC_RELAXED, __HIP_MEMORY_SCOPE_AGENT) != 0)) {
+                        if (lane == 0) {
+                            __hip_atomic_store(p.chain_status, 1, __ATOMIC_RELAXED, __HIP_MEMORY_SCOPE_AGENT);
+                            ctrl[CT_DRAIN] = 1;
+                        }
+                        break;
+                    }
+                }
+                __builtin_amdgcn_fence(__ATOMIC_ACQUIRE, "agent");
+                asm volatile("s_waitcnt vmcnt(0)" ::: "memory");
+            }
+            if (tid == 0 && !late) next_item_reg = atomicAdd(p.work_counter, 1u);
+        } else {
         if (!have_row) GLS_LOAD_ROW(phb, magb, run_t0 - lead + wave, GL_TB)
         have_row = false;
+        }
         for (int q = tid; q < acc_len + 128; q += GL_THREADS) {
 #pragma unroll
             for (int k = 0; k < NST; ++k) ringA[k * ring_floats + ring_len + q] = 0.f;
         }
         if (tid == 0) { ctrl[CT_OLA] = 0; ctrl[CT_OLB] = 0; ctrl[CT_OLB + 1] = 0; ctrl[CT_SNEXT] = (int)next_item_reg; }
         __syncthreads();
+        if (CHAIN) {
+            if (__builtin_amdgcn_readfirstlane(ctrl[CT_DRAIN])) break;
+            if (!have_row) GLS_LOAD_ROW(phb, magb, run_t0 - lead + wave, GL_TB)
+            have_row = false;
+        }
         int next_item = __builtin_amdgcn_readfirstlane(ctrl[CT_SNEXT]);
         int nb = b, nt0 = 0, nlen = 0, nslot = 0, nTb = p.T;
-        if (!late && next_item < p.n_items) decode_item(next_item, nb, nt0, nlen, nslot, nTb);
+        int nround = 0, npos = 0, nsp_lo = 0, nsp_hi = -1;
+        if (!late && next_item < n_total) {
+            decode_item(next_item, nb, nt0, nlen, nslot, nTb);
+            if (CHAIN) decode_chain(next_item, nround, npos, nsp_lo, nsp_hi);
+        }
 
         const int y_base_a = (run_t0 - lead) * hop - MH + fs;
         float mse_acc = 0.f;
@@ -411,7 +460,10 @@
                 int nv;
                 while ((nv = gl_flag_load(ctrl + CT_SNEXT)) == (int)GL_NO_ITEM) __builtin_amdgcn_s_sleep(1);
                 next_item = __builtin_amdgcn_readfirstlane(nv);
-                if (next_item < p.n_items) decode_item(next_item, nb, nt0, nlen, nslot, nTb);
+                if (next_item < n_total) {
+                    decode_item(next_item, nb, nt0, nlen, nslot, nTb);
+                    if (CHAIN) decode_chain(next_item, nround, npos, nsp_lo, nsp_hi);
+                }
             }
             GLS_URGENCY(i)
             cf v[16];
@@ -439,9 +491,17 @@
 #define GLS_NEXT_ROW()                                                                                                   \
             if (i + GL_NW < n_idx) {                                                                                     \
                 GLS_LOAD_ROW(phb, magb, t + GL_NW, GL_TB)                                                                \
-            } else if (next_item < p.n_items) {                                                                          \
-                GLS_LOAD_ROW(x_in + (size_t)nb * p.T * p.FP, p.mag + (size_t)nb * p.T * p.FP, nt0 - lead + wave, (RAG ? nTb : p.T)) \
+            } else if (next_item < n_total) {                                                                            \
+                    \
+                bool ready_ = true;                                                                                      \
+                if (CHAIN && nround > 0) {                                                                               \
+                    ready_ = span_ok(nsp_lo, nsp_hi, p.chain_base + (unsigned)nround);                                   \
+                    if (ready_) __builtin_amdgcn_fence(__ATOMIC_ACQUIRE, "agent");                                       \
+                }                                                                                                        \
+                if (ready_) {                                                                                            \
+                GLS_LOAD_ROW(GL_X_IN(nround) + (size_t)nb * p.T * p.FP, p.mag + (size_t)nb * p.T * p.FP, nt0 - lead + wave, (RAG ? nTb : p.T)) \
                 have_row = true;                                                                                         \
+                }                                                                                                        \
             }
             if (NST == 1) {
                 GLS_NEXT_ROW()
@@ -536,7 +596,7 @@
                 fft1024<FZ_LO, FZ_HI>(v, ex, tw, lane);
                 GLS_URGENCY(i + GL_NW)
                 if (MOM && MSE) mse_acc = 0.f;
-                gl_state_t* orow = x_out + ((size_t)b * p.T + tm) * p.FP;
+                gl_state_t* orow = GL_X_OUT(round) + ((size_t)b * p.T + tm) * p.FP;
                 gl_state_t* olo = orow + lane;
                 gl_state_t* ohi = orow + (MH - lane);
                 const cf xmid = merge_pass(v, [&](int c, cf x) {
@@ -585,9 +645,19 @@
                 for (int q = 1; q <= (slot >> 16); ++q) part[q] = 0.f;
             }
         }
+        if (CHAIN) asm volatile("s_waitcnt vmcnt(0)" ::: "memory");
         __syncthreads();
+        if (CHAIN && tid == 0 && round + 1 < p.chain_rounds) {
+            if (p.dbg_delay > 0 && (int)blockIdx.x == p.dbg_wg)
+                for (int q = 0; q < p.dbg_delay; ++q) __builtin_amdgcn_s_sleep(127);
+            __builtin_amdgcn_fence(__ATOMIC_RELEASE, "agent");
+            asm volatile("s_waitcnt vmcnt(0)" ::: "memory");
+            __hip_atomic_store(p.chain_done + pos, p.chain_base + (unsigned)round + 1u, __ATOMIC_RELAXED, __HIP_MEMORY_SCOPE_AGENT);
+        }
         item = next_item;
     }
+#undef GL_X_IN
+#undef GL_X_OUT
 #undef GLS_LOAD_ROW
 #undef GL_TB
 #undef GL_L
@@ -779,6 +849,27 @@
     return (int)items->size();
 }
 
+void gl_plan_spans(const std::vector<int4>& items, int win, int hop, int n_stage, std::vector<int4>* spans) {
+    const int halo = (win + hop - 1) / hop - 1;
+    const int wpad = (TTS_GL_NFFT - win) >> 1;
+    const int lag = (halo + 1) * hop > 2 * (TTS_GL_NFFT / 2 - wpad) ? halo : halo + 1;
+    const int reach = n_stage * lag;
+    const int n = (int)items.size();
+    std::vector<int> order((size_t)n);
+    for (int i = 0; i < n; ++i) order[i] = i;
+    std::sort(order.begin(), order.end(), [&](int a, int b) {
+        return items[a].x != items[b].x ? items[a].x < items[b].x : items[a].y < items[b].y;
+    });
+    spans->assign((size_t)n, make_int4(0, 0, -1, 0));
+    for (int q = 0; q < n; ++q) {
+        const int4& me = items[order[q]];
+        int lo = q, hi = q;
+        while (lo > 0 && items[order[lo - 1]].x == me.x && items[order[lo - 1]].y + items[order[lo - 1]].z - 1 >= me.y - reach) --lo;
+        while (hi + 1 < n && items[order[hi + 1]].x == me.x && items[order[hi + 1]].y <= me.y + me.z - 1 + reach) ++hi;
+        (*spans)[order[q]] = make_int4(q, lo, hi, 0);
+    }
+}
+
 hipError_t gl_plan_stream(GlParams& p, int n_workers, int n_stage, int force_runs, int force_run_len, hipStream_t stream) {
     struct Table { int4* ptr = nullptr; hipEvent_t ready = nullptr; hipStream_t owner = nullptr; bool seen = false; };
     struct Plan { std::vector<int4> items; int slots = 1, workers = 1; std::map<int, Table> dev; };
@@ -790,8 +881,12 @@
     p.ring_frames = gl_stream_ring_frames(p.win, p.hop, 1);
     const std::vector<int> key = {p.T, p.B, p.win, p.hop, n_workers, n_stage, force_runs, force_run_len};
     Plan& plan = cache[key];
-    if (plan.items.empty())
+    if (plan.items.empty()) {
+        std::vector<int4> spans;
         gl_plan_items(p.T, p.B, p.win, p.hop, n_workers, n_stage, force_runs, force_run_len, &plan.items, &plan.slots, &plan.workers);
+        gl_plan_spans(plan.items, p.win, p.hop, n_stage < 1 ? 1 : (n_stage > 3 ? 3 : n_stage), &spans);
+        plan.items.insert(plan.items.end(), spans.begin(), spans.end());
+    }
     int dev = 0;
     hipError_t e = hipGetDevice(&dev);
     if (e != hipSuccess) return e;
@@ -820,7 +915,8 @@
         else if (stream != t.owner && (e = hipStreamWaitEvent(stream, t.ready, 0)) != hipSuccess) return e;
     }
     p.items = t.ptr;
-    p.n_items = (int)plan.items.size();
+    p.n_items = (int)plan.items.size() / 2;
+    p.chain_span = t.ptr + p.n_items;
     p.slots_per_utt = plan.slots;
     p.n_workers = plan.workers;
     return hipSuccess;
@@ -886,9 +982,47 @@
     return hipErrorInvalidValue;
 }
 
+template <int W, int H, int NST>
+static hipError_t gl_stream_launch_chain_wh(hipStream_t s, const GlParams& p, dim3 grid, size_t lds) {
+    hipLaunchKernelGGL((gl_stream_kernel<0, W, H, false, NST, false, false, false, true>), grid, dim3(GL_THREADS), lds, s, p);
+    return hipGetLastError();
+}
+hipError_t launch_gl_stream_chain(hipStream_t s, const GlParams& p_in, int n_cus, int n_stage) {
+    GlParams p = p_in;
+    p.n_stage = n_stage;
+    p.ring_frames = gl_stream_ring_frames(p.win, p.hop, n_stage);
+    if (p.ring_frames < GL_NW || n_stage < 1 || n_stage > 3) return hipErrorInvalidValue;
+    if (p.chain_rounds < 2 || !p.chain_span || !p.chain_done || !p.chain_status || !p.phase_out) return hipErrorInvalidValue;
+    if (p.mse_partial || p.mom_c || p.n_frames || p.seeded) return hipErrorInvalidValue;
+    if ((long long)p.n_items * p.chain_rounds >= (long long)GL_NO_ITEM) return hipErrorInvalidValue;
+    const size_t lds = gl_stream_lds_bytes(p);
+    const int nwg = p.n_workers > 0 && p.n_workers < n_cus ? p.n_workers : (p.n_items < n_cus ? p.n_items : n_cus);
+    const dim3 grid(nwg);
+#define GLS_CHAIN_WH(W, H)                                                                   \
+    if (p.win == W && p.hop == H) {                                                          \
+        if (n_stage == 3) return gl_stream_launch_chain_wh<W, H, 3>(s, p, grid, lds);        \
+        if (n_stage == 2) return gl_stream_launch_chain_wh<W, H, 2>(s, p, grid, lds);        \
+        return gl_stream_launch_chain_wh<W, H, 1>(s, p, grid, lds);                          \
+    }
+    GLS_CHAIN_WH(1102, 275)
+    GLS_CHAIN_WH(800, 200)
+#undef GLS_CHAIN_WH
+    return hipErrorInvalidValue;
+}
+template <int W, int H, int NST>
+static hipError_t gl_stream_set_attr_chain() {
+    return hipFuncSetAttribute(reinterpret_cast<const void*>(&gl_stream_kernel<0, W, H, false, NST, false, false, false, true>),
+                               hipFuncAttributeMaxDynamicSharedMemorySize, 160 * 1024);
+}
+
 template <int W, int H, bool RAG>
 static hipError_t gl_stream_configure_wh() {
     hipError_t e;
+    if (!RAG) {
+        if ((e = gl_stream_set_attr_chain<W, H, 1>()) != hipSuccess) return e;
+        if ((e = gl_stream_set_attr_chain<W, H, 2>()) != hipSuccess) return e;
+        if ((e = gl_stream_set_attr_chain<W, H, 3>()) != hipSuccess) return e;
+    }
     if ((e = gl_stream_set_attr<0, W, H, true, 1, RAG>()) != hipSuccess) return e;
     if ((e = gl_stream_set_attr<0, W, H, false, 1, RAG>()) != hipSuccess) return e;
     if ((e = gl_stream_set_attr<0, W, H, false, 2, RAG>()) != hipSuccess) return e;
```
